# CIawevy/FreeFine

Hardware: NVIDIA B200
Metric: edits/s @512^2 50-step SD1.5 (FreeFine 2-D geometric edit) (higher is better)
Workload: dtype bf16

## Files before the change

freefine_b200/_lib.py:

```python
from __future__ import annotations

import ctypes as C
import os

_HERE = os.path.dirname(os.path.abspath(__file__))
LIB_PATH = os.environ.get("FREEFINE_B200_LIB", os.path.join(_HERE, "lib", "libfreefine_b200.so"))

FF_MAX_PASS = 4
FF_DT_F32, FF_DT_BF16, FF_DT_F16 = 0, 1, 2
FF_PASS_KEY_INVERT, FF_PASS_ROW_XOR, FF_PASS_ROW_WEIGHT, FF_PASS_KEY2_INVERT = 1, 2, 4, 8
FF_PASS_KEY_PREFIX, FF_PASS_KEY2_PREFIX = 16, 32


class FFAttnPass(C.Structure):
    _fields_ = [("kv_stream", C.c_int32), ("key_mask", C.c_int32), ("row_mask", C.c_int32), ("flags", C.c_uint32),
                ("weight", C.c_float), ("kv_stream2", C.c_int32), ("key_mask2", C.c_int32), ("reserved", C.c_int32)]


class FFAttnHeadPlan(C.Structure):
    _fields_ = [("n_pass", C.c_int32), ("reserved", C.c_int32 * 3), ("passes", FFAttnPass * FF_MAX_PASS)]


class FFAttnArgs(C.Structure):
    _fields_ = [("q", C.c_void_p), ("k", C.c_void_p), ("v", C.c_void_p), ("out", C.c_void_p), ("plan", C.c_void_p),
                ("bitmasks", C.c_void_p), ("mask_popcount", C.c_void_p),
                ("n_streams", C.c_int32), ("n_kv_streams", C.c_int32), ("heads", C.c_int32), ("head_dim", C.c_int32),
                ("s_q", C.c_int32), ("s_kv", C.c_int32), ("n_masks", C.c_int32), ("mask_words", C.c_int32),
                ("out_dtype", C.c_int32), ("scale", C.c_float), ("v_dtype", C.c_int32), ("v_head_stride", C.c_int32)]


PLAN_BYTES = C.sizeof(FFAttnHeadPlan)
PASS_BYTES = C.sizeof(FFAttnPass)

SIGNATURES = {
    "ff_version": (C.c_int, []),
    "ff_last_error": (C.c_char_p, []),
    "ff_attn_masked_kv": (C.c_int, [C.POINTER(FFAttnArgs), C.c_void_p]),
    "ff_attn_v_head_stride": (C.c_int, [C.c_int32]),
    "ff_attn_plain_smallkv": (C.c_int, [C.c_void_p] * 4 + [C.c_int32] * 5 + [C.c_float, C.c_int32, C.c_void_p]),
    "ff_debug_set_timeline": (C.c_int, [C.c_void_p]),
    "ff_kv_gather_cast": (C.c_int, [C.c_void_p, C.c_void_p, C.c_void_p, C.c_void_p, C.c_void_p, C.c_int32, C.c_int64,
                                    C.c_int32, C.c_int32, C.c_void_p]),
    "ff_mask_downsample_pack": (C.c_int, [C.c_void_p, C.c_int32, C.c_int32, C.c_int32, C.c_int32, C.c_int32,
                                          C.c_void_p, C.c_int32, C.c_void_p, C.c_void_p]),
    "ff_upsample2x_nhwc": (C.c_int, [C.c_void_p, C.c_void_p, C.c_int32, C.c_int32, C.c_int32, C.c_int32, C.c_void_p]),
    "ff_concat_nhwc": (C.c_int, [C.c_void_p, C.c_void_p, C.c_void_p, C.c_int64, C.c_int32, C.c_int32, C.c_void_p]),
    "ff_linear_bias_residual": (C.c_int, [C.c_void_p] * 5 + [C.c_int64, C.c_int32, C.c_int32, C.c_void_p, C.c_int64, C.c_void_p]),
    "ff_mask_prep": (C.c_int, [C.c_void_p] * 4 + [C.c_int32] * 7 + [C.c_void_p] * 6),
    "ff_dilate_mask": (C.c_int, [C.c_void_p, C.c_void_p, C.c_int32, C.c_int32, C.c_int32, C.c_int32, C.c_void_p]),
    "ff_warp_affine_blend": (C.c_int, [C.c_void_p, C.c_void_p, C.c_void_p, C.c_void_p, C.c_void_p, C.c_void_p,
                                       C.c_int32, C.c_int32, C.c_int32, C.c_int32, C.c_int32, C.c_int32, C.c_int32,
                                       C.c_int32, C.c_void_p]),
    "ff_ddim_cfg_step": (C.c_int, [C.c_void_p, C.c_void_p, C.c_void_p, C.c_void_p, C.c_void_p, C.c_float, C.c_float,
                                   C.c_float, C.c_float, C.c_float, C.c_float, C.c_float, C.c_void_p, C.c_void_p,
                                   C.c_int32, C.c_int32, C.c_int32, C.c_int32, C.c_void_p]),
    "ff_debug_set_trace": (C.c_int, [C.c_void_p]),
    "ff_ddim_step": (C.c_int, [C.c_void_p, C.c_void_p, C.c_void_p, C.c_void_p, C.c_float, C.c_float, C.c_float,
                               C.c_float, C.c_float, C.c_float, C.c_void_p, C.c_void_p, C.c_int32, C.c_int32,
                               C.c_int32, C.c_int32, C.c_void_p]),
    "ff_ddim_cfg_step_compose": (C.c_int, [C.c_void_p, C.c_int32, C.c_void_p, C.c_void_p, C.c_void_p, C.c_void_p,
                                           C.c_float, C.c_float, C.c_float, C.c_float, C.c_float, C.c_float, C.c_float,
                                           C.c_void_p, C.c_void_p, C.c_int32, C.c_int32, C.c_int32, C.c_int32, C.c_void_p]),
    "ff_ddim_inv_step": (C.c_int, [C.c_void_p, C.c_void_p, C.c_float, C.c_float, C.c_float, C.c_float, C.c_void_p,
                                   C.c_void_p, C.c_int64, C.c_void_p]),
    "ff_cross_region_blend": (C.c_int, [C.c_void_p, C.c_void_p, C.c_int32, C.c_void_p, C.c_int32, C.c_int32,
                                        C.c_int32, C.c_int32, C.c_void_p]),
    "ff_group_norm_ws_bytes": (C.c_int64, [C.c_int32, C.c_int32]),
    "ff_group_norm_nhwc": (C.c_int, [C.c_void_p, C.c_void_p, C.c_int64, C.c_void_p, C.c_void_p, C.c_void_p, C.c_void_p,
                                     C.c_int32, C.c_int32, C.c_int32, C.c_int32, C.c_float, C.c_int32, C.c_void_p]),
    "ff_bias_residual_nhwc": (C.c_int, [C.c_void_p, C.c_void_p, C.c_void_p, C.c_void_p, C.c_int64, C.c_int32,
                                        C.c_void_p]),
    "ff_geglu": (C.c_int, [C.c_void_p, C.c_void_p, C.c_int64, C.c_int32, C.c_void_p]),
    "ff_layer_norm": (C.c_int, [C.c_void_p, C.c_void_p, C.c_void_p, C.c_void_p, C.c_int64, C.c_int32, C.c_float,
                                C.c_void_p]),
}

_lib = None


def load() -> C.CDLL:
    global _lib
    if _lib is None:
        if not os.path.exists(LIB_PATH):
            raise RuntimeError(f"{LIB_PATH} is missing: build it with `python -m freefine_b200.csrc.build` "
                               "(freefine_b200 has no fallback path)")
        lib = C.CDLL(LIB_PATH)
        for name, (res, args) in SIGNATURES.items():
            fn = getattr(lib, name)
            fn.restype, fn.argtypes = res, args
        _lib = lib
    return _lib


def check(rc: int, what: str) -> None:
    if rc != 0:
        msg = load().ff_last_error()
        raise RuntimeError(f"{what} failed (code {rc}): {msg.decode() if msg else ''}")
```

freefine_b200/attention.py:

```python
from __future__ import annotations

import abc
import math

import os

import torch

from . import ops, plans


class AttentionControl(abc.ABC):
    def step_callback(self, x_t):
        return x_t

    def between_steps(self):
        return

    @property
    def num_uncond_att_layers(self):
        return self.num_att_layers if self.LOW_RESOURCE else 0

    @abc.abstractmethod
    def forward(self, attn, is_cross: bool, place_in_unet: str):
        raise NotImplementedError

    def _advance(self):
        self.cur_att_layer += 1
        if self.cur_att_layer == self.num_att_layers + self.num_uncond_att_layers:
            self.cur_att_layer = 0
            self.cur_step += 1
            self.between_steps()

    def __call__(self, attn, is_cross: bool, place_in_unet: str):
        self._advance()
        return attn

    def reset(self):
        self.cur_step = 0
        self.cur_att_layer = 0

    def __init__(self):
        self.cur_step = 0
        self.num_att_layers = -1
        self.cur_att_layer = 0
        self.LOW_RESOURCE = False


def _as_u8_stack(mask: torch.Tensor) -> torch.Tensor:
    m = mask if mask.dim() == 3 else mask[None]
    if m.dtype != torch.uint8:
        m = m.clamp(0, 255).to(torch.uint8)
    return m.contiguous()


class Attention_Modulator(AttentionControl):

    def __init__(self, start_layer=None):
        super().__init__()
        self.step_num = 0
        self.model_type = 'Inverse'
        self.use_cfg = False
        self.use_style_align = False
        self.use_tca = False
        self.local_edit = False
        self.fg_retain_mask = None
        self.fg_retain_mask_st2 = None
        self.fg_ref_mask = None
        self.obj_mask = None
        self.local_edit_region = None
        self.layer_idx = list(range(start_layer, 16)) if start_layer is not None else list(range(16))
        self.down_sampling_shape = dict()
        self.method = None
        self.context_guidance = None
        self.tca_scope = ['up']
        self.style_align_scope = ['down', 'mid', 'up']
        self.src_masks = None
        self.tgt_masks = None
        self.prompt_length = 1
        self.heads = None
        self.scale = None
        self.upcast_attention = False
        self.upcast_softmax = False
        self.log_mask = False
        self.sort_keys = True
        self.p_operand = "f16"
        self.small_kv_kernel = os.environ.get("FF_ATTN_SMALLKV", "1") != "0"
        self._tables = {}
        self._plans = {}

    def forward(self, attn, is_cross: bool, place_in_unet: str):
        return attn

    def reset(self):
        super().reset()
        self.step_num = 0
        self.model_type = 'Inverse'
        self.use_cfg = False
        self.use_tca = False
        self.use_style_align = False
        self.local_edit = False
        self.down_sampling_shape = dict()
        self.style_align = False
        self.method = None
        self.context_guidance = None
        self.tca_scope = ['up']
        self.style_align_scope = ['down', 'mid', 'up']
        self._tables.clear()
        self._plans.clear()

    def get_down_h_w(self, d_ratio, h, w, seq):
        if d_ratio in self.down_sampling_shape:
            nh, nw = self.down_sampling_shape[d_ratio]
            assert nh * nw == seq, f'{nh} * {nw} != {seq}'
            return nh, nw
        r = d_ratio // 8
        nh, nw = h // 8, w // 8
        while r != 1:
            r //= 2
            nh, nw = (nh + 1) // 2, (nw + 1) // 2
        assert nw * nh == seq
        self.down_sampling_shape[d_ratio] = [nh, nw]
        return nh, nw

    def _grid(self, H, W, seq):
        d_ratio = 2 ** int(math.log2((H * W // seq) ** 0.5) + 0.5)
        return self.get_down_h_w(d_ratio, H, W, seq)

    def _table(self, kind: str, seq: int, masks, min_tokens: int = 0):
        sig = tuple((m.data_ptr(), m._version, tuple(m.shape)) for m in masks)
        hit = self._tables.get((kind, seq))
        if hit is not None and hit[0] == sig:
            return hit[1], hit[2]
        stacks = [_as_u8_stack(m) for m in masks]
        E, H, W = stacks[0].shape
        for s in stacks:
            if s.shape != (E, H, W):
                raise ValueError(f"mask shapes differ: {[tuple(x.shape) for x in stacks]}")
            if not s.is_cuda:
                raise RuntimeError("controller masks must live on the CUDA device (no CPU path)")
        h, w = self._grid(H, W, seq)
        stacked = torch.stack(stacks, dim=1).reshape(E * len(stacks), H, W)
        words = ops.mask_words(max(seq, min_tokens))
        bits = torch.zeros((stacked.shape[0], words), dtype=torch.int32, device=stacked.device)
        bits, pop = ops.mask_downsample_pack(stacked, h, w, bits=bits)
        self._tables[(kind, seq)] = (sig, bits, pop, tuple(masks))
        return bits, pop

    def _plan(self, key, builder):
        p = self._plans.get(key)
        if p is None:
            if len(self._plans) > 256:
                self._plans.clear()
            host = builder()
            p = ops.to_device_bytes(host, self._device)
            self._plans[key] = p
            ops.PLAN_REGISTRY[p.data_ptr()] = host
        return p

    def _kv_index(self, kind: str, seq: int, bits, stream_masks):
        ck = (kind, "kvidx", seq)
        hit = self._tables.get(ck)
        if hit is not None and hit[0] is bits:
            return hit[1]
        shifts = torch.arange(32, device=bits.device, dtype=torch.int32)
        key_bits = ((bits[:, :, None] >> shifts) & 1).reshape(bits.shape[0], -1)[:, :seq]
        idx = plans.kv_sort_index(key_bits, stream_masks)
        self._tables[ck] = (bits, idx)
        return idx

    def _attend(self, query, key, value, plan, bits=None, pop=None, kv_index=None):
        self._device = query.device
        dt = query.dtype
        if dt not in (torch.float32, torch.bfloat16):
            query, key, value, dt = query.float(), key.float(), value.float(), torch.float32
        q = query.to(torch.bfloat16).contiguous()
        k = key.to(torch.bfloat16).contiguous()
        v = value.to(torch.bfloat16).contiguous()
        k, v = ops.kv_gather_cast(k, v, self.heads, kv_index, p_operand=self.p_operand)
        return ops.attn_masked_kv(q, k, v, plan, self.heads, self.scale, bits, pop, out_dtype=dt)

    def plain_attention(self, query, key, value):
        self._device = query.device
        B = query.shape[0]
        if key.shape[0] != B:
            raise ValueError("plain attention needs one K/V stream per query stream")
        d = query.shape[-1] // self.heads
        if (key.shape[1] <= (128 if d == 8 else ops.SMALLKV_MAX_KEYS) and d in ops.SMALLKV_HEAD_DIMS and self.p_operand == "f16"
                and self.small_kv_kernel):
            dt = query.dtype
            if dt not in (torch.float32, torch.bfloat16):
                query, key, value, dt = query.float(), key.float(), value.float(), torch.float32
            return ops.attn_plain_smallkv(query.to(torch.bfloat16).contiguous(), key.to(torch.bfloat16).contiguous(),
                                          value.to(torch.bfloat16).contiguous(), self.heads, self.scale, out_dtype=dt)
        plan = self._plan(("plain", B, self.heads), lambda: plans.plain_plan(B, self.heads))
        return self._attend(query, key, value, plan)

    def _tca_common(self, query, key, value, kind):
        B, S, _ = query.shape
        if self.cur_att_layer // 2 not in self.layer_idx:
            out = self.plain_attention(query, key, value)
            self._advance()
            return out
        if B % 4:
            raise ValueError(f"TCA expects 4 streams [u_e,u_r,c_e,c_r] per edit, got batch {B}")
        if self.method not in ('tca', 'mmsa'):
            raise ValueError(f"controller.method must be 'tca' or 'mmsa' here, got {self.method!r}")
        E = B // 4
        self._device = query.device
        if kind == "edit":
            bits, pop = self._table("edit", S, [self.fg_ref_mask, self.fg_retain_mask])
            src_id, tgt_id = (lambda e: 2 * e), (lambda e: 2 * e + 1)
        else:
            bits, pop = self._table("bg", S, [self.fg_retain_mask])
            src_id, tgt_id = (lambda e: e), (lambda e: e)
        if bits.shape[0] not in (2 * E if kind == "edit" else E,):
            raise ValueError(f"{E} edits in the stream batch but masks for {bits.shape[0]} rows")
        cg = None if self.method == 'mmsa' else float(self.context_guidance)
        pf = self.sort_keys
        plan = self._plan((kind, E, self.heads, self.method, cg, pf),
                          lambda: plans.tca_plan(E, self.heads, self.method, cg, src_id, tgt_id, kind=kind, prefix=pf))
        kv_index = None
        if pf:
            kv_index = self._kv_index(kind, S, bits, [src_id(s // 4) if s % 2 else -1 for s in range(B)])
        out = self._attend(query, key, value, plan, bits, pop, kv_index)
        self._advance()
        return out

    def Temporal_contextal_attention(self, query, key, value, is_cross, place_in_unet):
        return self._tca_common(query, key, value, "edit")

    def Temporal_contextal_attention_bg(self, query, key, value, is_cross, place_in_unet):
        return self._tca_common(query, key, value, "bg")

    def Temporal_contextal_attention_compose(self, query, key, value, is_cross, place_in_unet):
        B, S, _ = query.shape
        if self.cur_att_layer // 2 not in self.layer_idx:
            out = self.plain_attention(query, key, value)
            self._advance()
            return out
        N = B - 2
        self._device = query.device
        src = self.src_masks[:N] if torch.is_tensor(self.src_masks) else torch.stack(list(self.src_masks)[:N])
        tgt = self.tgt_masks[:N] if torch.is_tensor(self.tgt_masks) else torch.stack(list(self.tgt_masks)[:N])
        bits, pop = self._table("compose", S, [m for m in src] + [m for m in tgt])
        cg = None if self.method == 'mmsa' else float(self.context_guidance)
        pf = self.sort_keys
        plan = self._plan(("compose", N, self.heads, self.method, cg, pf),
                          lambda: plans.compose_plan(N, self.heads, self.method, cg, list(range(N)),
                                                     list(range(N, 2 * N)), prefix=pf))
        kv_index = self._kv_index("compose", S, bits, [-1] + list(range(N)) + [-1]) if pf else None
        out = self._attend(query, key, value, plan, bits, pop, kv_index)
        self._advance()
        return out

    def _style_align(self, query, key, value, mask, bg=False):
        B, S, _ = query.shape
        if B % 4:
            raise ValueError("style-align expects 4 streams per edit")
        E = B // 4
        self._device = query.device
        bits = pop = None
        src_id = None
        if self.method == 'sdsa':
            bits, pop = self._table("sdsa", S, [mask])
            src_id = lambda e: e
        pf = self.sort_keys and src_id is not None
        plan = self._plan(("style", E, self.heads, self.method, pf, bg),
                          lambda: plans.style_align_plan(E, self.heads, src_id, prefix=pf, bg=bg))
        kv_index = self._kv_index("sdsa", S, bits, [s // 4 if s % 2 else -1 for s in range(B)]) if pf else None
        out = self._attend(query, key, value, plan, bits, pop, kv_index)
        self._advance()
        return out

    def style_align_share_attention(self, query, key, value, is_cross, place_in_unet):
        return self._style_align(query, key, value, self.fg_ref_mask)

    def style_align_share_attention_bg(self, query, key, value, is_cross, place_in_unet):
        return self._style_align(query, key, value, self.fg_retain_mask, bg=True)

    def modulate_local_cross_attn(self, query, key, value, is_cross, place_in_unet):
        B, S, _ = query.shape
        if B % 4:
            raise ValueError("local cross-attention modulation expects 4 streams per edit")
        hs = self.plain_attention(query, key, value)
        bits, _ = self._table("region", S, [self.local_edit_region])
        ids = self._plans.get(("region_ids", B // 4))
        if ids is None:
            ids = torch.arange(B // 4, dtype=torch.int32, device=query.device)
            self._plans[("region_ids", B // 4)] = ids
        ops.cross_region_blend(hs, bits, ids)
        self._advance()
        return hs

    modulate_local_cross_attn_bg = modulate_local_cross_attn

    def modulate_local_cross_attn_compose(self, query, key, value, is_cross, place_in_unet):
        Bq, S, _ = query.shape
        self._device = query.device
        L = len(self.tgt_masks)
        nu = Bq - 1
        if key.shape[0] != nu + L:
            raise ValueError(f"expected {nu + L} prompt streams, got {key.shape[0]}")
        tg = self.tgt_masks if torch.is_tensor(self.tgt_masks) else torch.stack(list(self.tgt_masks))
        bits, pop = self._table("cross_compose", S, [m for m in tg], min_tokens=key.shape[1])

        def build():
            p = plans._empty(Bq, self.heads)
            for s in range(nu):
                for h in range(self.heads):
                    plans._add(p, s, h, s, 1.0)
            for h in range(self.heads):
                for i in range(L):
                    plans._add(p, nu, h, nu + i, 1.0, row_mask=i, flags=plans.FF_PASS_ROW_WEIGHT)
            return p

        plan = self._plan(("cross_compose", Bq, L, self.heads), build)
        out = self._attend(query, key, value, plan, bits, pop)
        self._advance()
        return out


def override_forward(unet):
    inner = unet.forward

    def forward(sample, timestep, encoder_hidden_states, *args, **kwargs):
        out = inner(sample, timestep, encoder_hidden_states, *args, **kwargs)
        if torch.is_tensor(out):
            return out
        return out.sample if hasattr(out, "sample") else out[0]

    return forward


class _DummyController:
    num_att_layers = 0
    use_tca = use_style_align = local_edit = False

    def __call__(self, *args):
        return args[0]


def _register(model, controller, flavour: str):
    if controller is None:
        controller = _DummyController()
    plain = Attention_Modulator()

    def ca_forward(self, place_in_unet):
        to_out = self.to_out[0] if isinstance(self.to_out, torch.nn.ModuleList) else self.to_out

        def forward(hidden_states, encoder_hidden_states=None, attention_mask=None, temb=None):
            is_cross = encoder_hidden_states is not None
            residual = hidden_states
            if self.spatial_norm is not None:
                hidden_states = self.spatial_norm(hidden_states, temb)
            input_ndim = hidden_states.ndim
            if input_ndim == 4:
                batch_size, channel, height, width = hidden_states.shape
                hidden_states = hidden_states.view(batch_size, channel, height * width).transpose(1, 2)
            if attention_mask is not None:
                raise NotImplementedError("explicit attention_mask is not part of the FreeFine hot path")
            if self.group_norm is not None:
                hidden_states = self.group_norm(hidden_states.transpose(1, 2)).transpose(1, 2)
            query = self.to_q(hidden_states)
            if encoder_hidden_states is None:
                encoder_hidden_states = hidden_states
            elif self.norm_cross:
                encoder_hidden_states = self.norm_encoder_hidden_states(encoder_hidden_states)
            key = self.to_k(encoder_hidden_states)
            value = self.to_v(encoder_hidden_states)

            c = controller if isinstance(controller, Attention_Modulator) else plain
            c.heads, c.scale = self.heads, self.scale
            c.upcast_attention, c.upcast_softmax = self.upcast_attention, self.upcast_softmax
            if flavour == "edit":
                if not is_cross and controller.use_style_align and place_in_unet in controller.style_align_scope:
                    hidden_states = controller.style_align_share_attention(query, key, value, is_cross, place_in_unet)
                elif not is_cross and controller.use_tca and place_in_unet in controller.tca_scope:
                    hidden_states = controller.Temporal_contextal_attention(query, key, value, is_cross, place_in_unet)
                elif controller.local_edit and is_cross:
                    hidden_states = controller.modulate_local_cross_attn(query, key, value, is_cross, place_in_unet)
                else:
                    hidden_states = c.plain_attention(query, key, value)
                    controller(None, is_cross, place_in_unet)
            elif flavour == "bggen":
                if place_in_unet in ['up'] and not is_cross and controller.use_tca:
                    hidden_states = controller.Temporal_contextal_attention_bg(query, key, value, is_cross, place_in_unet)
                elif controller.local_edit and is_cross:
                    hidden_states = controller.modulate_local_cross_attn_bg(query, key, value, is_cross, place_in_unet)
                else:
                    hidden_states = c.plain_attention(query, key, value)
                    controller(None, is_cross, place_in_unet)
            else:
                if not is_cross and controller.use_tca and place_in_unet in controller.tca_scope:
                    hidden_states = controller.Temporal_contextal_attention_compose(query, key, value, is_cross, place_in_unet)
                elif controller.local_edit and is_cross:
                    hidden_states = controller.modulate_local_cross_attn_compose(query, key, value, is_cross, place_in_unet)
                else:
                    hidden_states = c.plain_attention(query, key, value)
                    controller(None, is_cross, place_in_unet)

            block_res = getattr(self, "ff_block_residual", None)
            if (block_res is not None and input_ndim == 3 and hidden_states.is_cuda and hidden_states.dtype == torch.bfloat16
                    and isinstance(to_out, torch.nn.Linear) and not self.residual_connection
                    and self.rescale_output_factor == 1.0):
                self.ff_residual_fused = True
                return ops.linear_bias_residual(hidden_states.contiguous(), to_out.weight, to_out.bias, block_res)
            hidden_states = to_out(hidden_states)
            if input_ndim == 4:
                hidden_states = hidden_states.transpose(-1, -2).reshape(batch_size, channel, height, width)
            if self.residual_connection:
                hidden_states = hidden_states + residual
            if self.rescale_output_factor != 1.0:
                hidden_states = hidden_states / self.rescale_output_factor
            return hidden_states

        return forward

    def register_recr(net_, count, place_in_unet):
        if net_.__class__.__name__ == 'Attention':
            net_.forward = ca_forward(net_, place_in_unet)
            return count + 1
        if hasattr(net_, 'children'):
            for child in net_.children():
                count = register_recr(child, count, place_in_unet)
        return count

    n = 0
    for name, net in model.unet.named_children():
        if "down" in name:
            n += register_recr(net, 0, "down")
        elif "up" in name:
            n += register_recr(net, 0, "up")
        elif "mid" in name:
            n += register_recr(net, 0, "mid")
    controller.num_att_layers = n


def register_attention_control(model, controller):
    _register(model, controller, "edit")


def register_attention_control_4bggen(model, controller):
    _register(model, controller, "bggen")


def register_attention_control_compose(model, controller):
    _register(model, controller, "compose")
```

freefine_b200/csrc/cross_blend.cu:

```cuda
#include "ff_common.cuh"

namespace {

__global__ void __launch_bounds__(256)
cross_region_blend_kernel(uint4* __restrict__ hs, const uint32_t* __restrict__ bitmasks, int mask_words,
                          const int* __restrict__ region_mask, int n_edits, int S, int row_vec) {
  const long long per_stream = (long long)S * row_vec;
  const long long total = (long long)n_edits * per_stream;
  for (long long i = (long long)blockIdx.x * blockDim.x + threadIdx.x; i < total;
       i += (long long)gridDim.x * blockDim.x) {
    const int e = (int)(i / per_stream);
    const long long r = i - (long long)e * per_stream;
    const int tok = (int)(r / row_vec);
    const uint32_t word = __ldg(bitmasks + (size_t)__ldg(region_mask + e) * mask_words + (tok >> 5));
    const bool in_region = (word >> (tok & 31)) & 1u;
    uint4* base = hs + (long long)e * 4 * per_stream + r;
    const uint4 ur = base[per_stream];
    if (!in_region) base[2 * per_stream] = base[0];
    base[3 * per_stream] = ur;
  }
}

}

extern "C" int ff_cross_region_blend(void* hs, const uint32_t* bitmasks, int32_t mask_words,
                                     const int32_t* region_mask, int32_t n_edits, int32_t S, int32_t C, int32_t dtype,
                                     void* stream) {
  FF_REQUIRE(hs && bitmasks && region_mask, "ff_cross_region_blend: null pointer");
  FF_REQUIRE(n_edits > 0 && S > 0 && C > 0, "ff_cross_region_blend: bad shape");
  FF_REQUIRE(dtype == FF_DT_F32 || dtype == FF_DT_BF16, "ff_cross_region_blend: dtype must be f32 or bf16");
  const int es = dtype == FF_DT_F32 ? 4 : 2;
  FF_REQUIRE((C * es) % 16 == 0 && ff::aligned16(hs), "ff_cross_region_blend: rows must be 16-byte multiples");
  FF_REQUIRE(mask_words >= (S + 31) / 32, "ff_cross_region_blend: mask_words too small");
  const int row_vec = C * es / 16;
  const long long total = (long long)n_edits * S * row_vec;
  long long grid = (total + 255) / 256;
  if (grid > 148 * 8) grid = 148 * 8;
  cross_region_blend_kernel<<<(int)grid, 256, 0, static_cast<cudaStream_t>(stream)>>>(
      static_cast<uint4*>(hs), bitmasks, mask_words, region_mask, n_edits, S, row_vec);
  return ff::check_launch("ff_cross_region_blend");
}
```

freefine_b200/csrc/ddim_step.cu:

```cuda
#include "ff_common.cuh"

namespace {

struct StepCoef {
  float gs, sqrt_1m_at, sqrt_at, sqrt_ap, c_ddim, c_ddpm, sigma;
};

__device__ __forceinline__ void step_elem(float eu, float ec, float x, float nz, bool do_cfg, bool has_cfg_mask,
                                          uint8_t cfgm,
                                          uint8_t m, float sd, float cd, bool has_noise, const StepCoef& k,
                                          float& x_prev, float& x0) {
  float eps = eu;
  if (do_cfg) {
    float g = __fmul_rn(k.gs, __fsub_rn(ec, eu));
    if (has_cfg_mask) g = __fmul_rn(g, (float)cfgm);
    eps = __fadd_rn(eu, g);
  }
  x0 = __fdiv_rn(__fsub_rn(x, __fmul_rn(k.sqrt_1m_at, eps)), k.sqrt_at);
  const uint8_t om = (uint8_t)(1 - m);
  const float pdm = __fmul_rn(__fmul_rn(cd, eps), (float)m);
  const float dir = __fadd_rn(__fmul_rn(__fmul_rn(k.c_ddim, eps), (float)om), pdm);
  float xp = __fadd_rn(__fmul_rn(k.sqrt_ap, x0), dir);
  if (has_noise) xp = __fadd_rn(xp, __fmul_rn(__fmul_rn(sd, nz), (float)m));
  x_prev = xp;
}

template <int V>
__global__ void __launch_bounds__(256)
ddim_cfg_step_kernel(const float* __restrict__ eps4, const float* __restrict__ x, const float* __restrict__ noise,
                     const uint8_t* __restrict__ cfg_mask, const uint8_t* __restrict__ var_mask, StepCoef k,
                     float* __restrict__ x_prev, float* __restrict__ pred_x0, int n_edits, int C, int hw, int spe,
                     int so, int cs) {
  const int hwv = hw / V;
  const long long total = (long long)n_edits * so * C * hwv;
  for (long long i = (long long)blockIdx.x * blockDim.x + threadIdx.x; i < total;
       i += (long long)gridDim.x * blockDim.x) {
    const int p = (int)(i % hwv);
    long long r = i / hwv;
    const int c = (int)(r % C);
    r /= C;
    const int s = so == 2 ? (int)(r & 1) : 0;
    const int e = so == 2 ? (int)(r >> 1) : (int)r;
    const long long off_u = (((long long)(e * spe + s) * C + c) * hw) + (long long)p * V;
    const long long off_c = (((long long)(e * spe + s + cs) * C + c) * hw) + (long long)p * V;
    const long long off_x = (((long long)(e * so + s) * C + c) * hw) + (long long)p * V;
    const long long off_m = (long long)e * hw + (long long)p * V;
    float eu[V], ec[V], xv[V], nz[V], xp[V], x0[V];
    uint8_t cm[V], vm[V];
    if (V == 4) {
      *reinterpret_cast<float4*>(eu) = __ldg(reinterpret_cast<const float4*>(eps4 + off_u));
      *reinterpret_cast<float4*>(ec) = __ldg(reinterpret_cast<const float4*>(eps4 + off_c));
      *reinterpret_cast<float4*>(xv) = __ldg(reinterpret_cast<const float4*>(x + off_x));
      if (noise) *reinterpret_cast<float4*>(nz) = __ldg(reinterpret_cast<const float4*>(noise + off_x));
      if (cfg_mask) *reinterpret_cast<uint32_t*>(cm) = __ldg(reinterpret_cast<const uint32_t*>(cfg_mask + off_m));
      if (s == 0) *reinterpret_cast<uint32_t*>(vm) = __ldg(reinterpret_cast<const uint32_t*>(var_mask + off_m));
    } else {
      eu[0] = __ldg(eps4 + off_u);
      ec[0] = __ldg(eps4 + off_c);
      xv[0] = __ldg(x + off_x);
      if (noise) nz[0] = __ldg(noise + off_x);
      if (cfg_mask) cm[0] = __ldg(cfg_mask + off_m);
      if (s == 0) vm[0] = __ldg(var_mask + off_m);
    }
    const float sd = s == 0 ? k.sigma : 0.f;
    const float cd = s == 0 ? k.c_ddpm : k.c_ddim;
#pragma unroll
    for (int j = 0; j < V; ++j) {
      const uint8_t m = s == 0 ? vm[j] : (uint8_t)1;
      step_elem(eu[j], ec[j], xv[j], noise ? nz[j] : 0.f, cs != 0, cfg_mask != nullptr, cfg_mask ? cm[j] : (uint8_t)1,
                m, sd, cd, noise != nullptr, k, xp[j], x0[j]);
    }
    if (V == 4) {
      *reinterpret_cast<float4*>(x_prev + off_x) = *reinterpret_cast<float4*>(xp);
      if (pred_x0) *reinterpret_cast<float4*>(pred_x0 + off_x) = *reinterpret_cast<float4*>(x0);
    } else {
      x_prev[off_x] = xp[0];
      if (pred_x0) pred_x0[off_x] = x0[0];
    }
  }
}

template <int V>
__global__ void __launch_bounds__(256)
ddim_inv_step_kernel(const float* __restrict__ eps, const float* __restrict__ x, float sqrt_1m_at, float sqrt_at,
                     float sqrt_an, float c_next, float* __restrict__ x_next, float* __restrict__ pred_x0,
                     long long nv) {
  for (long long i = (long long)blockIdx.x * blockDim.x + threadIdx.x; i < nv;
       i += (long long)gridDim.x * blockDim.x) {
    float e[V], xv[V], xn[V], x0[V];
    if (V == 4) {
      *reinterpret_cast<float4*>(e) = __ldg(reinterpret_cast<const float4*>(eps) + i);
      *reinterpret_cast<float4*>(xv) = __ldg(reinterpret_cast<const float4*>(x) + i);
    } else {
      e[0] = __ldg(eps + i);
      xv[0] = __ldg(x + i);
    }
#pragma unroll
    for (int j = 0; j < V; ++j) {
      x0[j] = __fdiv_rn(__fsub_rn(xv[j], __fmul_rn(sqrt_1m_at, e[j])), sqrt_at);
      xn[j] = __fadd_rn(__fmul_rn(sqrt_an, x0[j]), __fmul_rn(c_next, e[j]));
    }
    if (V == 4) {
      reinterpret_cast<float4*>(x_next)[i] = *reinterpret_cast<float4*>(xn);
      if (pred_x0) reinterpret_cast<float4*>(pred_x0)[i] = *reinterpret_cast<float4*>(x0);
    } else {
      x_next[i] = xn[0];
      if (pred_x0) pred_x0[i] = x0[0];
    }
  }
}

inline int grid_for(long long work_items, int block) {
  long long need = (work_items + block - 1) / block;
  const long long cap = 148LL * 8;
  if (need > cap) need = cap;
  if (need < 1) need = 1;
  return (int)need;
}

}

static int launch_step(const char* what, const float* eps, int spe, int so, int cs, const float* x, const float* noise,
                       const uint8_t* cfg_mask, const uint8_t* var_mask, const StepCoef& k, float* x_prev,
                       float* pred_x0, int32_t n_edits, int32_t C, int32_t h, int32_t w, void* stream) {
  if (!(eps && x && var_mask && x_prev)) return ff::fail(FF_E_INVALID, "%s: null pointer", what);
  if (!(n_edits > 0 && C > 0 && h > 0 && w > 0))
    return ff::fail(FF_E_INVALID, "%s: bad shape %d,%d,%d,%d", what, n_edits, C, h, w);
  const int hw = h * w;
  cudaStream_t st = static_cast<cudaStream_t>(stream);
  const bool vec = (hw % 4 == 0) && ff::aligned16(eps) && ff::aligned16(x) && ff::aligned16(x_prev) &&
                   (!noise || ff::aligned16(noise)) && (!pred_x0 || ff::aligned16(pred_x0)) &&
                   (reinterpret_cast<uintptr_t>(var_mask) % 4 == 0) &&
                   (!cfg_mask || reinterpret_cast<uintptr_t>(cfg_mask) % 4 == 0);
  if (vec) {
    const long long items = (long long)n_edits * so * C * (hw / 4);
    ddim_cfg_step_kernel<4><<<grid_for(items, 256), 256, 0, st>>>(eps, x, noise, cfg_mask, var_mask, k, x_prev,
                                                                   pred_x0, n_edits, C, hw, spe, so, cs);
  } else {
    const long long items = (long long)n_edits * so * C * hw;
    ddim_cfg_step_kernel<1><<<grid_for(items, 256), 256, 0, st>>>(eps, x, noise, cfg_mask, var_mask, k, x_prev,
                                                                   pred_x0, n_edits, C, hw, spe, so, cs);
  }
  return ff::check_launch(what);
}

extern "C" int ff_ddim_cfg_step(const float* eps4, const float* x, const float* noise, const uint8_t* cfg_mask,
                                const uint8_t* var_mask, float guidance_scale, float sqrt_1m_at, float sqrt_at,
                                float sqrt_ap, float c_ddim, float c_ddpm, float sigma, float* x_prev,
                                float* pred_x0, int32_t n_edits, int32_t C, int32_t h, int32_t w, void* stream) {
  StepCoef k{guidance_scale, sqrt_1m_at, sqrt_at, sqrt_ap, c_ddim, c_ddpm, sigma};
  return launch_step("ff_ddim_cfg_step", eps4, 4, 2, 2, x, noise, cfg_mask, var_mask, k, x_prev, pred_x0, n_edits, C, h,
                     w, stream);
}

extern "C" int ff_ddim_step(const float* eps2, const float* x, const float* noise, const uint8_t* var_mask,
                            float sqrt_1m_at, float sqrt_at, float sqrt_ap, float c_ddim, float c_ddpm, float sigma,
                            float* x_prev, float* pred_x0, int32_t n_edits, int32_t C, int32_t h, int32_t w,
                            void* stream) {
  StepCoef k{0.f, sqrt_1m_at, sqrt_at, sqrt_ap, c_ddim, c_ddpm, sigma};
  return launch_step("ff_ddim_step", eps2, 2, 2, 0, x, noise, nullptr, var_mask, k, x_prev, pred_x0, n_edits, C, h, w,
                     stream);
}

extern "C" int ff_ddim_cfg_step_compose(const float* eps, int32_t streams_per_edit, const float* x, const float* noise,
                                        const uint8_t* cfg_mask, const uint8_t* var_mask, float guidance_scale,
                                        float sqrt_1m_at, float sqrt_at, float sqrt_ap, float c_ddim, float c_ddpm,
                                        float sigma, float* x_prev, float* pred_x0, int32_t n_edits, int32_t C, int32_t h,
                                        int32_t w, void* stream) {
  FF_REQUIRE(streams_per_edit >= 2, "ff_ddim_cfg_step_compose: streams_per_edit=%d < 2", streams_per_edit);
  StepCoef k{guidance_scale, sqrt_1m_at, sqrt_at, sqrt_ap, c_ddim, c_ddpm, sigma};
  return launch_step("ff_ddim_cfg_step_compose", eps, streams_per_edit, 1, streams_per_edit - 1, x, noise, cfg_mask,
                     var_mask, k, x_prev, pred_x0, n_edits, C, h, w, stream);
}

extern "C" int ff_ddim_inv_step(const float* eps, const float* x, float sqrt_1m_at, float sqrt_at, float sqrt_an,
                                float c_next, float* x_next, float* pred_x0, int64_t n, void* stream) {
  FF_REQUIRE(eps && x && x_next, "ff_ddim_inv_step: null pointer");
  FF_REQUIRE(n > 0, "ff_ddim_inv_step: n must be positive");
  cudaStream_t st = static_cast<cudaStream_t>(stream);
  const bool vec = (n % 4 == 0) && ff::aligned16(eps) && ff::aligned16(x) && ff::aligned16(x_next) &&
                   (!pred_x0 || ff::aligned16(pred_x0));
  if (vec) {
    ddim_inv_step_kernel<4><<<grid_for(n / 4, 256), 256, 0, st>>>(eps, x, sqrt_1m_at, sqrt_at, sqrt_an, c_next,
                                                                   x_next, pred_x0, n / 4);
  } else {
    ddim_inv_step_kernel<1><<<grid_for(n, 256), 256, 0, st>>>(eps, x, sqrt_1m_at, sqrt_at, sqrt_an, c_next, x_next,
                                                               pred_x0, n);
  }
  return ff::check_launch("ff_ddim_inv_step");
}
```

freefine_b200/ops.py:

```python
from __future__ import annotations

import contextlib
import ctypes as C
import os

import numpy as np
import torch

from . import _lib
from ._lib import FF_DT_BF16, FF_DT_F32

_DT = {torch.float32: FF_DT_F32, torch.bfloat16: FF_DT_BF16}

COUNTS: dict = {}
PROFILE = None
PLAN_REGISTRY: dict = {}


NVTX = os.environ.get("FREEFINE_NVTX", "0") == "1"


@contextlib.contextmanager
def nvtx_range(name: str):
    if NVTX and torch.cuda.is_available():
        torch.cuda.nvtx.range_push(name)
        try:
            yield
        finally:
            torch.cuda.nvtx.range_pop()
    else:
        yield


LIBRARY_ENTRIES = frozenset({"ff_linear_bias_residual"})


def _count(name: str):
    COUNTS[name] = COUNTS.get(name, 0) + 1


_RAW_STREAM = getattr(torch._C, "_cuda_getCurrentRawStream", None)


def _stream() -> C.c_void_p:
    if _RAW_STREAM is not None:
        return C.c_void_p(_RAW_STREAM(torch.cuda.current_device()))
    return C.c_void_p(torch.cuda.current_stream().cuda_stream)


def _ptr(t):
    return None if t is None else C.c_void_p(t.data_ptr())


def _chk(t: torch.Tensor, dtype, name: str, dims=None):
    if not t.is_cuda:
        raise RuntimeError(f"{name} must be a CUDA tensor (freefine_b200 has no CPU path)")
    if t.dtype != dtype:
        raise TypeError(f"{name} must be {dtype}, got {t.dtype}")
    if not t.is_contiguous():
        raise ValueError(f"{name} must be contiguous")
    if dims is not None and t.dim() != dims:
        raise ValueError(f"{name} must have {dims} dims, got {tuple(t.shape)}")
    return t


def ddim_cfg_step(eps4, x, noise, cfg_mask, var_mask, guidance_scale, sqrt_1m_at, sqrt_at, sqrt_ap, c_ddim, c_ddpm,
                  sigma, want_pred_x0=False, out=None):
    _chk(eps4, torch.float32, "eps4")
    _chk(x, torch.float32, "x")
    Cc, h, w = x.shape[-3:]
    n_edits = x.numel() // (2 * Cc * h * w)
    if eps4.numel() != 2 * x.numel():
        raise ValueError(f"eps4 {tuple(eps4.shape)} must hold 4 streams per edit for x {tuple(x.shape)}")
    _chk(var_mask, torch.uint8, "var_mask")
    if var_mask.numel() != n_edits * h * w:
        raise ValueError("var_mask must be [n_edits,h,w]")
    if cfg_mask is not None:
        _chk(cfg_mask, torch.uint8, "cfg_mask")
        if cfg_mask.numel() != n_edits * h * w:
            raise ValueError("cfg_mask must be [n_edits,h,w]")
    if noise is not None:
        _chk(noise, torch.float32, "noise")
        if noise.numel() != x.numel():
            raise ValueError("noise must have the shape of x")
    x_prev = torch.empty_like(x) if out is None else _chk(out, torch.float32, "out")
    x0 = torch.empty_like(x) if want_pred_x0 else None
    lib = _lib.load()
    rc = lib.ff_ddim_cfg_step(_ptr(eps4), _ptr(x), _ptr(noise), _ptr(cfg_mask), _ptr(var_mask), guidance_scale,
                              sqrt_1m_at, sqrt_at, sqrt_ap, c_ddim, c_ddpm, sigma, _ptr(x_prev), _ptr(x0), n_edits,
                              Cc, h, w, _stream())
    _lib.check(rc, "ff_ddim_cfg_step")
    _count("ff_ddim_cfg_step")
    return (x_prev, x0) if want_pred_x0 else x_prev


def ddim_step(eps2, x, noise, var_mask, sqrt_1m_at, sqrt_at, sqrt_ap, c_ddim, c_ddpm, sigma, want_pred_x0=False):
    _chk(eps2, torch.float32, "eps2")
    _chk(x, torch.float32, "x")
    if eps2.shape != x.shape:
        raise ValueError("eps2 and x must have the same shape")
    Cc, h, w = x.shape[-3:]
    n_edits = x.numel() // (2 * Cc * h * w)
    _chk(var_mask, torch.uint8, "var_mask")
    if var_mask.numel() != n_edits * h * w:
        raise ValueError("var_mask must be [n_edits,h,w]")
    if noise is not None:
        _chk(noise, torch.float32, "noise")
    x_prev = torch.empty_like(x)
    x0 = torch.empty_like(x) if want_pred_x0 else None
    rc = _lib.load().ff_ddim_step(_ptr(eps2), _ptr(x), _ptr(noise), _ptr(var_mask), sqrt_1m_at, sqrt_at, sqrt_ap,
                                  c_ddim, c_ddpm, sigma, _ptr(x_prev), _ptr(x0), n_edits, Cc, h, w, _stream())
    _lib.check(rc, "ff_ddim_step")
    _count("ff_ddim_step")
    return (x_prev, x0) if want_pred_x0 else x_prev


def ddim_cfg_step_compose(eps, streams_per_edit, x, noise, cfg_mask, var_mask, guidance_scale, sqrt_1m_at, sqrt_at,
                          sqrt_ap, c_ddim, c_ddpm, sigma):
    _chk(eps, torch.float32, "eps")
    _chk(x, torch.float32, "x")
    Cc, h, w = x.shape[-3:]
    E = x.numel() // (Cc * h * w)
    if eps.numel() != E * streams_per_edit * Cc * h * w:
        raise ValueError("eps must hold streams_per_edit streams per edit")
    _chk(var_mask, torch.uint8, "var_mask")
    if cfg_mask is not None:
        _chk(cfg_mask, torch.uint8, "cfg_mask")
    if noise is not None:
        _chk(noise, torch.float32, "noise")
    x_prev = torch.empty_like(x)
    rc = _lib.load().ff_ddim_cfg_step_compose(_ptr(eps), streams_per_edit, _ptr(x), _ptr(noise), _ptr(cfg_mask), _ptr(var_mask),
                                              guidance_scale, sqrt_1m_at, sqrt_at, sqrt_ap, c_ddim, c_ddpm, sigma,
                                              _ptr(x_prev), None, E, Cc, h, w, _stream())
    _lib.check(rc, "ff_ddim_cfg_step_compose")
    _count("ff_ddim_cfg_step_compose")
    return x_prev


def ddim_inv_step(eps, x, sqrt_1m_at, sqrt_at, sqrt_an, c_next, want_pred_x0=False):
    _chk(eps, torch.float32, "eps")
    _chk(x, torch.float32, "x")
    if eps.shape != x.shape:
        raise ValueError("eps and x must have the same shape")
    x_next = torch.empty_like(x)
    x0 = torch.empty_like(x) if want_pred_x0 else None
    rc = _lib.load().ff_ddim_inv_step(_ptr(eps), _ptr(x), sqrt_1m_at, sqrt_at, sqrt_an, c_next, _ptr(x_next), _ptr(x0),
                                      x.numel(), _stream())
    _lib.check(rc, "ff_ddim_inv_step")
    _count("ff_ddim_inv_step")
    return (x_next, x0) if want_pred_x0 else x_next


def warp_affine_blend(src, theta, dsize=None, mask_src=None, bg=None, mode="bilinear", want_mask=False, out=None):
    if src.dtype not in _DT:
        raise TypeError(f"src must be float32 or bfloat16, got {src.dtype}")
    _chk(src, src.dtype, "src", 4)
    N, Cc, H, W = src.shape
    dW, dH = (W, H) if dsize is None else dsize
    theta = theta.to(device=src.device, dtype=torch.float32)
    if theta.dim() == 2:
        theta = theta[None].expand(N, 2, 3)
    theta = theta.contiguous()
    if theta.shape != (N, 2, 3):
        raise ValueError(f"theta must be [N,2,3], got {tuple(theta.shape)}")
    if mask_src is not None:
        _chk(mask_src, torch.uint8, "mask_src")
        if mask_src.numel() != N * H * W:
            raise ValueError("mask_src must be [N,H,W]")
        if bg is None:
            raise ValueError("mask_src needs a background")
        _chk(bg, src.dtype, "bg", 4)
        if bg.shape != (N, Cc, dH, dW):
            raise ValueError("bg must be [N,C,dH,dW]")
    if out is None:
        out = torch.empty((N, Cc, dH, dW), dtype=src.dtype, device=src.device)
    else:
        _chk(out, src.dtype, "out", 4)
        if out.shape != (N, Cc, dH, dW):
            raise ValueError("out must be [N,C,dH,dW]")
    mask_out = torch.empty((N, dH, dW), dtype=torch.uint8, device=src.device) if (want_mask and mask_src is not None) else None
    rc = _lib.load().ff_warp_affine_blend(_ptr(src), _ptr(theta), _ptr(mask_src), _ptr(bg), _ptr(out), _ptr(mask_out),
                                          N, Cc, H, W, dH, dW, 0 if mode == "bilinear" else 1, _DT[src.dtype],
                                          _stream())
    _lib.check(rc, "ff_warp_affine_blend")
    _count("ff_warp_affine_blend")
    return (out, mask_out) if want_mask else out


def mask_words(S: int) -> int:
    return (S + 31) // 32


def mask_downsample_pack(masks, h, w, bits=None, popcount=None):
    _chk(masks, torch.uint8, "masks", 3)
    n, H, W = masks.shape
    words = mask_words(h * w)
    if bits is None:
        bits = torch.empty((n, words), dtype=torch.int32, device=masks.device)
    if popcount is None:
        popcount = torch.empty((n,), dtype=torch.int32, device=masks.device)
    rc = _lib.load().ff_mask_downsample_pack(_ptr(masks), n, H, W, h, w, _ptr(bits), bits.shape[1], _ptr(popcount),
                                             _stream())
    _lib.check(rc, "ff_mask_downsample_pack")
    _count("ff_mask_downsample_pack")
    return bits, popcount


def mask_prep(shifted, ori, draw, cons, lat_hw, use_auto_draw, reduce_inp_artifacts):
    _chk(shifted, torch.uint8, "shifted", 3)
    _chk(ori, torch.uint8, "ori", 3)
    E, H, W = shifted.shape
    for name, t in (("ori", ori), ("draw", draw), ("cons", cons)):
        if t is not None:
            _chk(t, torch.uint8, name, 3)
            if tuple(t.shape) != (E, H, W):
                raise ValueError(f"{name} must be [{E},{H},{W}], got {tuple(t.shape)}")
    h, w = lat_hw
    dev = shifted.device
    fg, sh, orib = (torch.empty((E, H, W), dtype=torch.uint8, device=dev) for _ in range(3))
    comp, lvar = (torch.empty((E, h, w), dtype=torch.uint8, device=dev) for _ in range(2))
    rc = _lib.load().ff_mask_prep(_ptr(shifted), _ptr(ori), _ptr(draw), _ptr(cons), E, H, W, h, w, int(bool(use_auto_draw)),
                                  int(bool(reduce_inp_artifacts)), _ptr(fg), _ptr(sh), _ptr(orib), _ptr(comp), _ptr(lvar), _stream())
    _lib.check(rc, "ff_mask_prep")
    _count("ff_mask_prep")
    return fg, sh, orib, comp, lvar


def dilate_mask(mask, k):
    m = mask if mask.dim() == 3 else mask[None]
    _chk(m, torch.uint8, "mask", 3)
    out = torch.empty_like(m)
    rc = _lib.load().ff_dilate_mask(_ptr(m), _ptr(out), m.shape[0], m.shape[1], m.shape[2], int(k), _stream())
    _lib.check(rc, "ff_dilate_mask")
    _count("ff_dilate_mask")
    return out if mask.dim() == 3 else out[0]


class StagedV:
    __slots__ = ("data", "heads", "head_dim")

    def __init__(self, data, heads, head_dim):
        self.data, self.heads, self.head_dim = data, heads, head_dim

    def values(self):
        return self.data[..., : self.head_dim].reshape(self.data.shape[0], self.data.shape[1], -1)


P_OPERAND_DTYPE = {"f16": torch.float16, "bf16x2": torch.bfloat16}


def kv_gather_cast(k, v, heads, row_index=None, gather_k=True, p_operand="f16"):
    _chk(k, torch.bfloat16, "k", 3)
    _chk(v, torch.bfloat16, "v", 3)
    if v.shape != k.shape or k.shape[2] % heads:
        raise ValueError("k and v must have the same shape [Bk,Skv,heads*d]")
    Bk, Sk, Ck = k.shape
    d = Ck // heads
    if row_index is not None:
        _chk(row_index, torch.int64, "row_index", 1)
        if row_index.numel() != Bk * Sk:
            raise ValueError("row_index must hold one source row per K/V row")
    lib = _lib.load()
    vhs = lib.ff_attn_v_head_stride(d)
    do_k = gather_k and row_index is not None
    k_out = torch.empty_like(k) if do_k else None
    vdt = P_OPERAND_DTYPE[p_operand]
    v_out = torch.empty((Bk, Sk, heads, vhs), dtype=vdt, device=v.device)
    rc = lib.ff_kv_gather_cast(_ptr(k) if do_k else None, _ptr(v), _ptr(row_index), _ptr(k_out), _ptr(v_out),
                               _lib.FF_DT_F16 if vdt == torch.float16 else FF_DT_BF16, Bk * Sk, heads, d, _stream())
    _lib.check(rc, "ff_kv_gather_cast")
    _count("ff_kv_gather_cast")
    return (k_out if do_k else k), StagedV(v_out, heads, d)


def attn_masked_kv(q, k, v, plan, heads, scale, bitmasks=None, popcount=None, out_dtype=None, out=None,
                   p_operand="f16"):
    _chk(q, torch.bfloat16, "q", 3)
    _chk(k, torch.bfloat16, "k", 3)
    B, Sq, Cc = q.shape
    Bk, Skv, Ck = k.shape
    if Ck != Cc or Cc % heads:
        raise ValueError(f"bad shapes q{tuple(q.shape)} k{tuple(k.shape)} heads={heads}")
    if not isinstance(v, StagedV):
        _chk(v, torch.bfloat16, "v", 3)
        if v.shape != k.shape:
            raise ValueError(f"bad shapes k{tuple(k.shape)} v{tuple(v.shape)}")
        v = kv_gather_cast(k, v, heads, None, p_operand=p_operand)[1]
    vt = v.data
    _chk(vt, vt.dtype if vt.dtype in (torch.float16, torch.bfloat16) else torch.float16, "v", 4)
    if tuple(vt.shape[:3]) != (Bk, Skv, heads) or v.head_dim * heads != Ck:
        raise ValueError(f"staged V {tuple(vt.shape)} does not match k{tuple(k.shape)} heads={heads}")
    _chk(plan, torch.uint8, "plan")
    if plan.numel() != B * heads * _lib.PLAN_BYTES:
        raise ValueError(f"plan holds {plan.numel()} bytes, expected {B * heads * _lib.PLAN_BYTES}")
    out_dtype = torch.bfloat16 if out_dtype is None else out_dtype
    if out is None:
        out = torch.empty((B, Sq, Cc), dtype=out_dtype, device=q.device)
    else:
        _chk(out, out_dtype, "out", 3)
    a = _lib.FFAttnArgs()
    a.q, a.k, a.v, a.out, a.plan = q.data_ptr(), k.data_ptr(), vt.data_ptr(), out.data_ptr(), plan.data_ptr()
    if bitmasks is not None:
        _chk(bitmasks, torch.int32, "bitmasks", 2)
        _chk(popcount, torch.int32, "popcount", 1)
        a.bitmasks, a.mask_popcount = bitmasks.data_ptr(), popcount.data_ptr()
        a.n_masks, a.mask_words = bitmasks.shape[0], bitmasks.shape[1]
    else:
        a.bitmasks, a.mask_popcount, a.n_masks, a.mask_words = None, None, 0, 0
    a.n_streams, a.n_kv_streams, a.heads, a.head_dim = B, Bk, heads, Cc // heads
    a.s_q, a.s_kv = Sq, Skv
    a.out_dtype = _DT[out_dtype]
    a.scale = float(scale)
    a.v_dtype = _lib.FF_DT_F16 if vt.dtype == torch.float16 else FF_DT_BF16
    a.v_head_stride = vt.shape[3]
    prof = PROFILE
    if prof is not None:
        ev0, ev1 = torch.cuda.Event(enable_timing=True), torch.cuda.Event(enable_timing=True)
        ev0.record()
    with nvtx_range(f"ff_attn_masked_kv S_q={Sq} S_kv={Skv} d={Cc // heads} streams={B}"):
        rc = _lib.load().ff_attn_masked_kv(C.byref(a), _stream())
    _lib.check(rc, "ff_attn_masked_kv")
    COUNTS["ff_attn_masked_kv"] = COUNTS.get("ff_attn_masked_kv", 0) + 1
    if prof is not None:
        ev1.record()
        prof.append(dict(ev0=ev0, ev1=ev1, B=B, Bk=Bk, s_q=Sq, s_kv=Skv, d=Cc // heads, heads=heads, plan=PLAN_REGISTRY.get(plan.data_ptr()),
                         popcount=popcount))
    return out


SMALLKV_MAX_KEYS = 256
SMALLKV_HEAD_DIMS = (8, 40, 80, 160)


def attn_plain_smallkv(q, k, v, heads, scale, out_dtype=None):
    _chk(q, torch.bfloat16, "q", 3)
    _chk(k, torch.bfloat16, "k", 3)
    _chk(v, torch.bfloat16, "v", 3)
    B, Sq, Cc = q.shape
    if k.shape[0] != B or k.shape[2] != Cc or v.shape != k.shape or Cc % heads:
        raise ValueError(f"bad shapes q{tuple(q.shape)} k{tuple(k.shape)} v{tuple(v.shape)} heads={heads}")
    out_dtype = torch.bfloat16 if out_dtype is None else out_dtype
    out = torch.empty((B, Sq, Cc), dtype=out_dtype, device=q.device)
    with nvtx_range(f"ff_attn_plain_smallkv S_q={Sq} S_kv={k.shape[1]} d={Cc // heads} streams={B}"):
        rc = _lib.load().ff_attn_plain_smallkv(_ptr(q), _ptr(k), _ptr(v), _ptr(out), B, heads, Cc // heads, Sq, k.shape[1],
                                               float(scale), _DT[out_dtype], _stream())
    _lib.check(rc, "ff_attn_plain_smallkv")
    _count("ff_attn_plain_smallkv")
    return out


def cross_region_blend(hs, bitmasks, region_ids):
    if hs.dtype not in _DT:
        raise TypeError("hs must be float32 or bfloat16")
    _chk(hs, hs.dtype, "hs", 3)
    B, S, Cc = hs.shape
    if B % 4:
        raise ValueError("hs must hold 4 streams per edit")
    _chk(bitmasks, torch.int32, "bitmasks", 2)
    _chk(region_ids, torch.int32, "region_ids", 1)
    rc = _lib.load().ff_cross_region_blend(_ptr(hs), _ptr(bitmasks), bitmasks.shape[1], _ptr(region_ids), B // 4, S, Cc,
                                           _DT[hs.dtype], _stream())
    _lib.check(rc, "ff_cross_region_blend")
    _count("ff_cross_region_blend")
    return hs


def _nhwc_view(x: torch.Tensor, name: str):
    if not x.is_cuda:
        raise RuntimeError(f"{name} must be a CUDA tensor (freefine_b200 has no CPU path)")
    if x.dtype != torch.bfloat16:
        raise TypeError(f"{name} must be bfloat16, got {x.dtype}")
    if x.dim() != 4:
        raise ValueError(f"{name} must be [N,C,H,W], got {tuple(x.shape)}")
    if not x.permute(0, 2, 3, 1).is_contiguous():
        raise ValueError(f"{name} must be dense channels_last (NHWC) memory")
    N, Cc, H, W = x.shape
    return N, H * W, Cc


_GN_WS: dict = {}


def _gn_workspace(N: int, G: int, device) -> torch.Tensor:
    key = (device, _stream().value)
    need = int(_lib.load().ff_group_norm_ws_bytes(N, G))
    ws = _GN_WS.get(key)
    if ws is None or ws.numel() < need:
        ws = torch.zeros(max(need, 1 << 20), dtype=torch.uint8, device=device)
        _GN_WS[key] = ws
    return ws


def group_norm_nhwc(x, gamma, beta, groups, eps, add_nc=None, silu=False):
    N, HW, Cc = _nhwc_view(x, "x")
    _chk(gamma, torch.bfloat16, "gamma", 1)
    _chk(beta, torch.bfloat16, "beta", 1)
    if gamma.numel() != Cc or beta.numel() != Cc:
        raise ValueError("gamma / beta must have C elements")
    add_ld = Cc
    if add_nc is not None:
        if not add_nc.is_cuda or add_nc.dtype != torch.float32 or add_nc.dim() != 2:
            raise TypeError("add_nc must be a 2-D float32 CUDA tensor")
        if tuple(add_nc.shape) != (N, Cc) or add_nc.stride(1) != 1 or (N > 1 and add_nc.stride(0) < Cc):
            raise ValueError(f"add_nc must be [{N},{Cc}] with unit column stride, got {tuple(add_nc.shape)} {add_nc.stride()}")
        add_ld = add_nc.stride(0) if N > 1 else Cc
    y = torch.empty_like(x)
    ws = _gn_workspace(N, groups, x.device)
    rc = _lib.load().ff_group_norm_nhwc(_ptr(x), _ptr(add_nc), add_ld, _ptr(gamma), _ptr(beta), _ptr(y), _ptr(ws), N, HW, Cc,
                                        groups, float(eps), int(bool(silu)), _stream())
    _lib.check(rc, "ff_group_norm_nhwc")
    _count("ff_group_norm_nhwc")
    return y


def bias_residual_nhwc(h, bias=None, res=None):
    N, HW, Cc = _nhwc_view(h, "h")
    if bias is not None:
        _chk(bias, torch.bfloat16, "bias", 1)
        if bias.numel() != Cc:
            raise ValueError("bias must have C elements")
    if res is not None:
        if _nhwc_view(res, "res") != (N, HW, Cc):
            raise ValueError("res must have the shape of h")
    rc = _lib.load().ff_bias_residual_nhwc(_ptr(h), _ptr(bias), _ptr(res), _ptr(h), N * HW, Cc, _stream())
    _lib.check(rc, "ff_bias_residual_nhwc")
    _count("ff_bias_residual_nhwc")
    return h


def upsample2x_nhwc(x):
    N, HW, Cc = _nhwc_view(x, "x")
    H, W = x.shape[2], x.shape[3]
    y = torch.empty((N, Cc, 2 * H, 2 * W), dtype=x.dtype, device=x.device, memory_format=torch.channels_last)
    rc = _lib.load().ff_upsample2x_nhwc(_ptr(x), _ptr(y), N, H, W, Cc, _stream())
    _lib.check(rc, "ff_upsample2x_nhwc")
    _count("ff_upsample2x_nhwc")
    return y


def concat_nhwc(a, b):
    N, HW, Ca = _nhwc_view(a, "a")
    Nb, HWb, Cb = _nhwc_view(b, "b")
    if (N, HW) != (Nb, HWb) or a.shape[2:] != b.shape[2:]:
        raise ValueError(f"concat_nhwc: shapes {tuple(a.shape)} and {tuple(b.shape)} differ outside the channel dimension")
    out = torch.empty((N, Ca + Cb, a.shape[2], a.shape[3]), dtype=a.dtype, device=a.device, memory_format=torch.channels_last)
    rc = _lib.load().ff_concat_nhwc(_ptr(a), _ptr(b), _ptr(out), N * HW, Ca, Cb, _stream())
    _lib.check(rc, "ff_concat_nhwc")
    _count("ff_concat_nhwc")
    return out


_LT_WS: dict = {}


def linear_bias_residual(x, weight, bias=None, res=None, out=None):
    _chk(x, torch.bfloat16, "x")
    _chk(weight, torch.bfloat16, "weight", 2)
    N, K = weight.shape
    if x.shape[-1] != K:
        raise ValueError(f"x has {x.shape[-1]} features, weight expects {K}")
    M = x.numel() // K
    if bias is not None:
        _chk(bias, torch.bfloat16, "bias", 1)
        if bias.numel() != N:
            raise ValueError("bias must have N elements")
    oshape = tuple(x.shape[:-1]) + (N,)
    if res is not None:
        _chk(res, torch.bfloat16, "res")
        if tuple(res.shape) != oshape:
            raise ValueError(f"res must be {oshape}, got {tuple(res.shape)}")
    if out is None:
        out = torch.empty(oshape, dtype=torch.bfloat16, device=x.device)
    else:
        _chk(out, torch.bfloat16, "out")
        if tuple(out.shape) != oshape:
            raise ValueError(f"out must be {oshape}, got {tuple(out.shape)}")
    key = (x.device, _stream().value)
    ws = _LT_WS.get(key)
    if ws is None:
        ws = _LT_WS[key] = torch.empty(32 << 20, dtype=torch.uint8, device=x.device)
    rc = _lib.load().ff_linear_bias_residual(_ptr(x), _ptr(weight), _ptr(bias), _ptr(res), _ptr(out), M, N, K, _ptr(ws),
                                             ws.numel(), _stream())
    _lib.check(rc, "ff_linear_bias_residual")
    _count("ff_linear_bias_residual")
    return out


def geglu(h):
    _chk(h, torch.bfloat16, "h")
    F2 = h.shape[-1]
    if F2 % 2:
        raise ValueError("last dim must be even")
    M = h.numel() // F2
    out = torch.empty(*h.shape[:-1], F2 // 2, dtype=h.dtype, device=h.device)
    rc = _lib.load().ff_geglu(_ptr(h), _ptr(out), M, F2 // 2, _stream())
    _lib.check(rc, "ff_geglu")
    _count("ff_geglu")
    return out


def layer_norm(x, gamma, beta, eps):
    _chk(x, torch.bfloat16, "x")
    Cc = x.shape[-1]
    _chk(gamma, torch.bfloat16, "gamma", 1)
    _chk(beta, torch.bfloat16, "beta", 1)
    if gamma.numel() != Cc or beta.numel() != Cc:
        raise ValueError("gamma / beta must have C elements")
    y = torch.empty_like(x)
    rc = _lib.load().ff_layer_norm(_ptr(x), _ptr(gamma), _ptr(beta), _ptr(y), x.numel() // Cc, Cc, float(eps), _stream())
    _lib.check(rc, "ff_layer_norm")
    _count("ff_layer_norm")
    return y


def to_device_bytes(arr: np.ndarray, device) -> torch.Tensor:
    t = torch.from_numpy(np.ascontiguousarray(arr).view(np.uint8).reshape(-1))
    if torch.cuda.is_available():
        t = t.pin_memory()
    return t.to(device, non_blocking=True)
```

freefine_b200/pipeline.py:

```python
from __future__ import annotations

from copy import deepcopy

import numpy as np
import torch
import torch.nn.functional as F

from . import ops
from .attention import (Attention_Modulator, override_forward, register_attention_control,
                        register_attention_control_4bggen, register_attention_control_compose)


def randn_tensor(shape, generator=None, device=None, dtype=None):
    return torch.randn(tuple(shape), generator=generator, device=device, dtype=dtype)


def seed_everything(seed):
    torch.manual_seed(seed)
    np.random.seed(seed % (2 ** 32))
    return seed


class FreeFinePipeline:

    def __init__(self, unet, vae, tokenizer, text_encoder, scheduler, controller=None, device=None):
        self.unet, self.vae, self.tokenizer = unet, vae, tokenizer
        self.text_encoder, self.scheduler = text_encoder, scheduler
        self.controller = controller
        self._device = torch.device(device) if device is not None else next(unet.parameters()).device
        self.method_type = None

    @classmethod
    def from_parts(cls, parts, controller=None, device=None):
        return cls(parts.unet, parts.vae, parts.tokenizer, parts.text_encoder, parts.scheduler, controller, device)

    @property
    def device(self):
        return self._device

    def modify_unet_forward(self):
        self.unet.forward = override_forward(self.unet)

    def _ratio(self):
        return self.scheduler.config.num_train_timesteps // self.scheduler.num_inference_steps

    def _get_variance(self, timestep, prev_timestep):
        a_t = self.scheduler.alphas_cumprod[timestep]
        a_prev = self.scheduler.alphas_cumprod[prev_timestep] if prev_timestep >= 0 else self.scheduler.final_alpha_cumprod
        return ((1 - a_prev) / (1 - a_t)) * (1 - a_t / a_prev)

    def _ctrl_coefs(self, timestep, eta):
        t = int(timestep)
        prev_t = t - self._ratio()
        a_t = self.scheduler.alphas_cumprod[t]
        a_prev = self.scheduler.alphas_cumprod[prev_t] if prev_t > 0 else self.scheduler.final_alpha_cumprod
        std = eta * self._get_variance(t, prev_t).to(torch.float32) ** 0.5
        stdt = torch.cat((std[None,], torch.zeros_like(std)[None,]))
        c_ddpm = ((1 - a_prev - stdt ** 2) ** 0.5)[0]
        return dict(sqrt_1m_at=float((1 - a_t) ** 0.5), sqrt_at=float(a_t ** 0.5), sqrt_ap=float(a_prev ** 0.5),
                    c_ddim=float((1 - a_prev) ** 0.5), c_ddpm=float(c_ddpm), sigma=float(std))

    def _inv_coefs(self, timestep):
        nxt = int(timestep)
        t = min(nxt - self._ratio(), 999)
        a_t = self.scheduler.alphas_cumprod[t] if t >= 0 else self.scheduler.final_alpha_cumprod
        a_next = self.scheduler.alphas_cumprod[nxt]
        return dict(sqrt_1m_at=float((1 - a_t) ** 0.5), sqrt_at=float(a_t ** 0.5), sqrt_an=float(a_next ** 0.5),
                    c_next=float((1 - a_next) ** 0.5))

    def inv_step(self, model_output, timestep, x, eta=0., verbose=False):
        return ops.ddim_inv_step(model_output.float().contiguous(), x.float().contiguous(), want_pred_x0=True,
                                 **self._inv_coefs(timestep))

    def _var_mask(self, mask, n_edits, h, w):
        m = mask
        if m.dtype != torch.uint8:
            raise TypeError(f"ctrl_step mask must be uint8 (reference quirk Q2), got {m.dtype}")
        m = m.reshape(-1, h, w)
        if m.shape[0] == 1 and n_edits > 1:
            m = m.expand(n_edits, h, w)
        if m.shape[0] != n_edits:
            raise ValueError(f"mask for {m.shape[0]} edits, latents for {n_edits}")
        return m.contiguous().to(self.device)

    def ctrl_step(self, model_output, timestep, x, mask, eta: float = 0.0, generator=None):
        if model_output.shape[0] % 2 or mask is None:
            raise NotImplementedError("ctrl_step mirrors the 2-stream [edit, ref] local-DDPM form of the reference")
        E = model_output.shape[0] // 2
        h, w = x.shape[-2:]
        noise = None
        if eta > 0:
            noise = randn_tensor(model_output.shape, generator=generator, device=model_output.device,
                                 dtype=torch.float32).contiguous()
        return ops.ddim_step(model_output.float().contiguous(), x.float().contiguous(), noise,
                             self._var_mask(mask, E, h, w), want_pred_x0=True, **self._ctrl_coefs(timestep, eta))

    def cfg_ctrl_step(self, noise_pred4, timestep, x, cfg_mask, var_mask, guidance_scale, eta=0.0, generator=None):
        E = x.shape[0] // 2
        h, w = x.shape[-2:]
        noise = None
        if eta > 0:
            if isinstance(generator, (list, tuple)):
                if len(generator) != E:
                    raise ValueError(f"{len(generator)} generators for {E} edits")
                noise = torch.stack([randn_tensor((2,) + tuple(x.shape[1:]), generator=g, device=x.device, dtype=torch.float32)
                                     for g in generator]).reshape(x.shape).contiguous()
            else:
                noise = randn_tensor(x.shape, generator=generator, device=x.device, dtype=torch.float32).contiguous()
        cm = None if cfg_mask is None else self._var_mask(cfg_mask, E, h, w)
        return ops.ddim_cfg_step(noise_pred4.float().contiguous(), x.float().contiguous(), noise, cm,
                                 self._var_mask(var_mask, E, h, w), float(guidance_scale),
                                 **self._ctrl_coefs(timestep, eta))

    def linear_param(self, t, t1, t0, t2, end_scale=0.5):
        if t < t1 or t > t2:
            raise ValueError(f"t must be in [{t1}, {t2}]")
        if t <= t0:
            return 1 + (end_scale - 1) / (t0 - t1) * (t - t1)
        return end_scale + (-end_scale / (t2 - t0)) * (t - t0)

    def preprocess_image(self, image, device):
        image = torch.from_numpy(image).float() / 127.5 - 1
        return image.permute(2, 0, 1).unsqueeze(0).to(device)

    @torch.no_grad()
    def image2latent(self, image):
        if isinstance(image, np.ndarray):
            if image.dtype == np.uint8:
                image = image.astype(np.float32) / 255.0 * 2 - 1
            image = torch.from_numpy(image)
        tensor = image.clone().detach()
        if tensor.ndim == 3:
            tensor = tensor.permute(2, 0, 1).unsqueeze(0)
        elif tensor.ndim != 4:
            raise ValueError(f"Invalid tensor shape: {tensor.shape}")
        tensor = tensor.to(device=self.device, dtype=next(self.vae.parameters()).dtype)
        return self.vae.encode(tensor)['latent_dist'].mean * 0.18215

    @torch.no_grad()
    def latent2image(self, latents, return_type='np'):
        latents = 1 / 0.18215 * latents.detach()
        image = self.vae.decode(latents.to(next(self.vae.parameters()).dtype))['sample']
        image = (image.float() / 2 + 0.5).clamp(0, 1)
        if return_type == 'np':
            image = (image.cpu().permute(0, 2, 3, 1).numpy()[0] * 255).astype(np.uint8)
        return image

    @torch.no_grad()
    def get_text_embeddings(self, prompt):
        ids = self.tokenizer(prompt, padding="max_length", max_length=77, return_tensors="pt").input_ids
        return self.text_encoder(ids.to(self.device))[0]

    def _unet(self, latents, t, text_embeddings):
        dt = self.unet.dtype if hasattr(self.unet, "dtype") else next(self.unet.parameters()).dtype
        if latents.is_cuda and not (torch.is_tensor(t) and t.is_cuda):
            t = torch.full((), int(t), dtype=torch.int64, device=latents.device)
        with ops.nvtx_range(f"ff.unet streams={latents.shape[0]}"):
            out = self.unet(latents.to(dt), t, encoder_hidden_states=text_embeddings.to(dt))
        return out.float()

    @torch.no_grad()
    def invert(self, image, prompt, num_inference_steps=50, num_actual_inference_steps=None, guidance_scale=7.5,
               eta=0.0, return_intermediates=False, verbose=False, **kwds):
        batch_size = image.shape[0]
        if isinstance(prompt, list):
            if batch_size == 1:
                image = image.expand(len(prompt), -1, -1, -1)
        elif isinstance(prompt, str) and batch_size > 1:
            prompt = [prompt] * batch_size
        text_embeddings = self.get_text_embeddings(prompt)
        latents = self.image2latent(image).float()
        if guidance_scale > 1.:
            uncond = self.get_text_embeddings([""] * batch_size)
            text_embeddings = torch.cat([uncond, text_embeddings], dim=0)
            self.controller.use_cfg = True
        self.scheduler.set_timesteps(num_inference_steps)
        latents_list = [latents]
        for i, t in enumerate(reversed(self.scheduler.timesteps)):
            if num_actual_inference_steps is not None and i >= num_actual_inference_steps:
                continue
            with ops.nvtx_range(f"ff.invert step {i} t={int(t)}"):
                model_inputs = torch.cat([latents] * 2) if guidance_scale > 1. else latents
                noise_pred = self._unet(model_inputs, t, text_embeddings)
                if guidance_scale > 1.:
                    eu, ec = noise_pred.chunk(2, dim=0)
                    noise_pred = eu + guidance_scale * (ec - eu)
                latents, _ = self.inv_step(noise_pred, t, latents)
            latents_list.append(latents)
        if return_intermediates:
            return latents, latents_list
        return latents

    @torch.no_grad()
    def forward_sampling(self, prompt, prompt_embeds=None, refer_latents=None, batch_size=1, end_step=None,
                         height=512, width=512, num_inference_steps=50, num_actual_inference_steps=None,
                         guidance_scale=7.5, latents=None, unconditioning=None, neg_prompt=None,
                         return_intermediates=False, eta=0.0, end_scale=0.5, local_var_reg=None,
                         completion_mask_cfg=None, local_edit_text=True, share_attn=True, method_type=None,
                         verbose=False, local_perturbation=True, generator=None, **kwds):
        self.method_type = method_type
        assert guidance_scale > 1.0, 'USING THIS MODULE CFG Must > 1.0'
        c = self.controller
        if share_attn:
            if method_type == 'tca':
                c.use_tca, c.layer_idx, c.method = True, list(range(10, 16)), 'tca'
            elif method_type in ('mmsa', 'mmsa_es'):
                c.use_tca, c.layer_idx, c.method = True, list(range(10, 16)), 'mmsa'
            elif method_type == 'ssa':
                c.use_style_align, c.method = True, 'ssa'
            elif method_type == 'sdsa':
                c.use_style_align, c.method = True, 'sdsa'
        c.use_cfg = True
        c.local_edit = local_edit_text
        if prompt_embeds is None:
            if isinstance(prompt, str) and batch_size > 1:
                prompt = [prompt] * batch_size
            cond = self.get_text_embeddings(prompt)
        else:
            cond = prompt_embeds
        n2 = cond.shape[0]
        if n2 % 2:
            raise ValueError("forward_sampling expects [edit_prompt, \"\"] pairs")
        E = n2 // 2
        if latents is None:
            latents = torch.randn((n2, self.unet.in_channels, height // 8, width // 8), device=self.device)
        uncond = self.get_text_embeddings([neg_prompt if neg_prompt else ""] * n2)
        text_embeddings = torch.cat([uncond.reshape(E, 2, *uncond.shape[1:]), cond.reshape(E, 2, *cond.shape[1:])],
                                    dim=1).reshape(4 * E, *cond.shape[1:])
        self.scheduler.set_timesteps(num_inference_steps)
        latents = latents.float().clone()
        latents_list = [latents]
        if num_actual_inference_steps is None:
            num_actual_inference_steps = num_inference_steps
        start_step = num_inference_steps - num_actual_inference_steps
        C, h, w = latents.shape[1:]
        var_mask = local_var_reg if local_perturbation else torch.ones_like(local_var_reg)
        for i, t in enumerate(self.scheduler.timesteps):
            if i < start_step:
                continue
            ref_latent = refer_latents[i - start_step + 1].reshape(E, 2, C, h, w)[:, 1]
            if latents.shape[0] == 2 * E:
                latents = latents.clone()
                latents.view(E, 2, C, h, w)[:, 1] = ref_latent
            else:
                latents = torch.stack([latents.reshape(E, C, h, w), ref_latent], 1).reshape(2 * E, C, h, w)
            if method_type == 'tca':
                c.context_guidance = self.linear_param(i, start_step, end_step, num_inference_steps, end_scale=end_scale)
            elif method_type == 'mmsa_es' and i >= end_step:
                c.use_tca = False
            lat = latents.view(E, 2, C, h, w)
            model_inputs = torch.cat([lat, lat], dim=1).reshape(4 * E, C, h, w)
            te = text_embeddings
            if unconditioning is not None and isinstance(unconditioning, list):
                te = text_embeddings.clone().reshape(E, 4, *cond.shape[1:])
                te[:, :2] = unconditioning[i].to(te.dtype)
                te = te.reshape(4 * E, *cond.shape[1:])
            c.log_mask = False
            with ops.nvtx_range(f"ff.sample step {i} t={int(t)}"):
                noise_pred = self._unet(model_inputs, t, te)
                latents = self.cfg_ctrl_step(noise_pred, t, latents, completion_mask_cfg if local_edit_text else None,
                                             var_mask, guidance_scale, eta=eta, generator=generator)
            latents_list.append(latents)
        image = self.latent2image(latents, return_type="pt")
        if return_intermediates:
            return image, latents_list
        return image, None

    def mask_reduce_dim(self, mask):
        return mask[:, :, 0] if mask.ndim == 3 else mask

    def dilate_mask(self, mask, dilate_factor=15):
        k = int(dilate_factor)
        a = k // 2
        m = torch.from_numpy(np.ascontiguousarray(mask.astype(np.uint8))).to(self.device)
        squeeze = m.dim() == 2
        if m.is_cuda and m.shape[1] % 4 == 0 and int(m.max()) <= 1:
            y = ops.dilate_mask(m if squeeze else m.permute(2, 0, 1).contiguous(), k)
            return (y if squeeze else y.permute(1, 2, 0)).cpu().numpy()
        x = (m[None, None] if squeeze else m.permute(2, 0, 1)[None]).float()
        x = F.pad(x, (a, k - 1 - a, a, k - 1 - a), value=0.0)
        y = F.max_pool2d(x, kernel_size=k, stride=1)
        y = y[0, 0] if squeeze else y[0].permute(1, 2, 0)
        return y.to(torch.uint8).cpu().numpy()

    def prepare_tensor_mask(self, mask, sup_res_w, sup_res_h, binary=True):
        if mask.ndim == 3:
            mask = mask[:, :, 0]
        t = torch.tensor(mask, device=self.device)[None, None]
        t = F.interpolate(t, (sup_res_h, sup_res_w), mode="nearest").squeeze(0).squeeze(0)
        if binary:
            t[t > 0.0] = 1.0
        else:
            norm_ = t.max()
            t = t.float()
            t /= norm_
        return t

    def _masks_for_kernel(self, masks, sup_res_w, sup_res_h, init_code):
        if self.device.type != 'cuda':
            return None
        lh, lw = init_code.shape[2], init_code.shape[3]
        if sup_res_h % lh or sup_res_w % lw or sup_res_w % 4:
            return None
        out = []
        for m in masks:
            if m is None:
                out.append(None)
                continue
            m = np.asarray(m)
            m = m[:, :, 0] if m.ndim == 3 else m
            if m.shape != (sup_res_h, sup_res_w) or m.dtype.kind not in 'ub':
                return None
            out.append(torch.from_numpy(np.ascontiguousarray(m.astype(np.uint8)))[None].to(self.device))
        return out

    def prepare_various_mask(self, shifted_mask, ori_mask, draw_mask, sup_res_w, sup_res_h, init_code, verbose=False,
                             use_auto_draw=False, cons_area=None, reduce_inp_artifacts=False):
        if use_auto_draw or reduce_inp_artifacts:
            assert cons_area is not None, 'for auto draw / auto artifact expansion use cons area '
        dev_masks = self._masks_for_kernel((shifted_mask, ori_mask, None if use_auto_draw else draw_mask,
                                            cons_area if (use_auto_draw or reduce_inp_artifacts) else None),
                                           sup_res_w, sup_res_h, init_code)
        if dev_masks is not None:
            r = ops.mask_prep(*dev_masks, (init_code.shape[2], init_code.shape[3]), use_auto_draw, reduce_inp_artifacts)
            return tuple(t[0] for t in r)
        P = lambda m: self.prepare_tensor_mask(m, sup_res_w, sup_res_h)
        if not use_auto_draw:
            if not reduce_inp_artifacts:
                sh, ori = P(shifted_mask), P(ori_mask)
                flex = P(draw_mask) * (1 - sh)
                fg = flex + sh
                fg[fg > 0] = 1.0
                comp, lvar = flex, flex
            else:
                assert cons_area is not None, 'for auto artifact expansion use cons area '
                dil = P(self.dilate_mask(ori_mask, 30))
                cons, sh, ori = P(cons_area), P(shifted_mask), P(ori_mask)
                flex = P(draw_mask) * (1 - sh)
                fg = flex + sh
                fg[fg > 0] = 1.0
                comp = flex
                lvar = (1 - cons) * (1 - sh) * dil + flex
                lvar[lvar > 0] = 1
        else:
            assert cons_area is not None, 'for auto draw better use cons area '
            if not reduce_inp_artifacts:
                dil_t = P(self.dilate_mask(shifted_mask, 15))
                sh, ori, cons = P(shifted_mask), P(ori_mask), P(cons_area)
                fg = sh
                cons = cons - ori
                comp = (1 - cons) * (1 - sh) * dil_t
                lvar = comp
            else:
                dil_t = P(self.dilate_mask(shifted_mask, 15))
                dil = P(self.dilate_mask(ori_mask, 30))
                sh, ori, cons = P(shifted_mask), P(ori_mask), P(cons_area)
                fg = sh
                cons = cons - ori
                comp = dil + dil_t
                comp[comp > 0] = 1
                comp *= (1 - cons) * (1 - sh)
                lvar = comp
        size = (init_code.shape[2], init_code.shape[3])
        comp = F.interpolate(comp[None, None], size, mode='nearest').squeeze(0).squeeze(0)
        lvar = F.interpolate(lvar[None, None], size, mode='nearest').squeeze(0).squeeze(0)
        return fg, sh, ori, comp, lvar

    @torch.no_grad()
    def DDIM_inversion_func(self, img, mask, prompt, num_step, start_step=0, ref_img=None, verbose=False):
        source_image = self.preprocess_image(img, self.device)
        if ref_img is not None:
            source_image = torch.cat((source_image, self.preprocess_image(ref_img, self.device)))
        if mask.ndim == 3:
            mask = mask[:, :, 0]
        latents, latents_list = self.invert(source_image, prompt, guidance_scale=1.0, num_inference_steps=num_step,
                                            num_actual_inference_steps=num_step - start_step,
                                            return_intermediates=True, verbose=verbose)
        self.controller.reset()
        return np.asarray(mask, dtype=np.float32), latents_list

    def Details_Preserving_regeneration(self, source_image, inverted_latents, edit_prompt, shifted_mask, ori_mask,
                                        draw_mask, num_steps=100, start_step=30, end_step=10, eta=1,
                                        guidance_scale=7.5, share_attn=True, method_type='tca', verbose=False,
                                        local_text_edit=True, local_perturbation=True, return_intermediates=False,
                                        use_auto_draw=False, cons_area=None, use_share_attention=False,
                                        reduce_inp_artifacts=False, end_scale=0.5):
        start_latents = inverted_latents[-1]
        init_code_orig = deepcopy(start_latents)
        full_h, full_w = source_image.shape[:2]
        fg_retain, fg_retain_st2, fg_ref, comp_cfg, local_var = self.prepare_various_mask(
            shifted_mask, ori_mask, draw_mask, full_h, full_w, init_code_orig, verbose=verbose,
            use_auto_draw=use_auto_draw, cons_area=cons_area, reduce_inp_artifacts=reduce_inp_artifacts)
        c = self.controller
        c.fg_retain_mask = fg_retain.to(self.device)
        c.fg_retain_mask_st2 = fg_retain_st2.to(self.device)
        c.fg_ref_mask = fg_ref.to(self.device)
        c.local_edit_region = fg_retain.to(self.device)
        c.reset()
        c.log_mask = False
        gen_images, intermediates = self.forward_sampling(
            prompt=[edit_prompt, ""], refer_latents=inverted_latents[::-1], end_step=end_step, batch_size=2,
            latents=init_code_orig, guidance_scale=guidance_scale, num_inference_steps=num_steps,
            num_actual_inference_steps=num_steps - start_step, eta=eta, completion_mask_cfg=comp_cfg,
            local_var_reg=local_var, share_attn=share_attn, method_type=method_type, verbose=verbose,
            blending=local_text_edit, local_perturbation=local_perturbation, return_intermediates=return_intermediates,
            use_share_attention=use_share_attention, end_scale=end_scale)
        edit_gen_image, ref_gen_image = gen_images
        c.reset()
        to_u8 = lambda im: (im.permute(1, 2, 0).detach().cpu().numpy() * 255).astype(np.uint8)
        return to_u8(edit_gen_image), to_u8(ref_gen_image), intermediates

    def FreeFine_generation(self, ori_img, ori_mask, coarse_input, target_mask, guidance_text, guidance_scale, eta,
                            end_step=10, num_step=50, start_step=25, share_attn=True, method_type='tca',
                            local_text_edit=True, local_perturbation=True, verbose=True, return_ori=False, seed=42,
                            draw_mask=None, return_intermediates=False, use_auto_draw=False, cons_area=None,
                            reduce_inp_artifacts=False, end_scale=0.5):
        methods = ['tca', 'ssa', 'sdsa', 'mmsa', 'mmsa_es']
        assert method_type in methods, f"check method type f{method_type}, which is not in {methods}"
        seed_everything(seed)
        ori_mask = self.mask_reduce_dim(ori_mask)
        target_mask = self.mask_reduce_dim(target_mask)
        if draw_mask is not None:
            draw_mask = self.mask_reduce_dim(draw_mask)
        shifted_mask, inverted_latent = self.DDIM_inversion_func(img=coarse_input, mask=target_mask, prompt="",
                                                                 num_step=num_step, start_step=start_step,
                                                                 ref_img=ori_img, verbose=verbose)
        edit_img, ref_img, intermediates = self.Details_Preserving_regeneration(
            coarse_input, inverted_latent, guidance_text, target_mask, ori_mask, draw_mask, num_steps=num_step,
            start_step=start_step, end_step=end_step, guidance_scale=guidance_scale, eta=eta, share_attn=share_attn,
            method_type=method_type, verbose=verbose, local_text_edit=local_text_edit,
            local_perturbation=local_perturbation, return_intermediates=return_intermediates, cons_area=cons_area,
            use_auto_draw=use_auto_draw, end_scale=end_scale, reduce_inp_artifacts=reduce_inp_artifacts)
        self.last_intermediates = intermediates
        if not return_ori:
            return edit_img
        return edit_img, ref_img


    def prepare_mask_bggen(self, mask, sup_res_w, sup_res_h, init_code):
        mask_tensor = self.prepare_tensor_mask(mask, sup_res_w, sup_res_h)
        lvar = F.interpolate(mask_tensor[None, None], (init_code.shape[2], init_code.shape[3]), mode='nearest')
        return mask_tensor, lvar.squeeze(0).squeeze(0)

    @torch.no_grad()
    def forward_sampling_background_gen(self, prompt, batch_size=1, end_step=None, height=512, width=512,
                                        num_inference_steps=50, num_actual_inference_steps=None, guidance_scale=7.5,
                                        latents=None, refer_latents=None, unconditioning=None, neg_prompt=None,
                                        return_intermediates=False, eta=0.0, local_var_reg=None, local_cfg_reg=None,
                                        local_text_edit=True, share_attn=True, method_type='tca', verbose=False,
                                        local_perturbation=True, end_scale=0.5, latent_blended=True,
                                        blend_range=(0, 40), **kwds):
        assert guidance_scale > 1.0, 'USING THIS MODULE CFG Must > 1.0'
        self.method_type = method_type
        c = self.controller
        if share_attn:
            if method_type == 'tca':
                c.use_tca, c.layer_idx, c.method = True, list(range(10, 16)), 'tca'
            elif method_type in ('mmsa', 'mmsa_es'):
                c.use_tca, c.layer_idx, c.method = True, list(range(10, 16)), 'mmsa'
            elif method_type == 'ssa':
                c.use_style_align, c.method = True, 'ssa'
            elif method_type == 'sdsa':
                c.use_style_align, c.method = True, 'sdsa'
        c.use_cfg = True
        c.local_edit = local_text_edit
        if isinstance(prompt, str) and batch_size > 1:
            prompt = [prompt] * batch_size
        cond = self.get_text_embeddings(prompt)
        n2 = cond.shape[0]
        E = n2 // 2
        uncond = self.get_text_embeddings([neg_prompt if neg_prompt else ""] * n2)
        text_embeddings = torch.cat([uncond.reshape(E, 2, *uncond.shape[1:]), cond.reshape(E, 2, *cond.shape[1:])],
                                    dim=1).reshape(4 * E, *cond.shape[1:])
        self.scheduler.set_timesteps(num_inference_steps)
        if num_actual_inference_steps is None:
            num_actual_inference_steps = num_inference_steps
        start_step = num_inference_steps - num_actual_inference_steps
        C, h, w = latents.shape[1:]
        edit = latents.float().reshape(-1, C, h, w)[:E] if latents.shape[0] == E else latents.float().reshape(E, -1, C, h, w)[:, 0]
        latents_list = [latents]
        var_mask = local_var_reg if local_perturbation else torch.ones_like(local_var_reg)
        for i, t in enumerate(self.scheduler.timesteps):
            if i < start_step:
                continue
            ref = refer_latents[i - start_step].float().reshape(E, C, h, w)
            lat = torch.stack([edit, ref], dim=1)
            if method_type == 'tca':
                c.context_guidance = self.linear_param(i, start_step, end_step, num_inference_steps, end_scale=end_scale)
            elif method_type == 'mmsa_es' and i >= end_step:
                c.use_tca = False
            model_inputs = torch.cat([lat, lat], dim=1).reshape(4 * E, C, h, w)
            c.log_mask = False
            noise_pred = self._unet(model_inputs, t, text_embeddings)
            out = self.cfg_ctrl_step(noise_pred, t, lat.reshape(2 * E, C, h, w), local_cfg_reg if local_text_edit else None,
                                     var_mask, guidance_scale, eta=eta)
            edit = out.reshape(E, 2, C, h, w)[:, 0]
            latents_list.append(edit if E > 1 else edit[0])
            last = out
        image = self.latent2image(last, return_type="pt")
        if return_intermediates:
            return image, latents_list
        return image, None

    def Details_Preserving_regeneration_background(self, ori_img, inverted_latents, edit_prompt, ori_mask, num_steps=100,
                                                   start_step=30, end_step=10, guidance_scale=3.5, eta=1, verbose=False,
                                                   local_text_edit=True, local_perturbation=True, end_scale=0.5,
                                                   return_intermediates=False, share_attn=True, method_type='tca',
                                                   latent_blended=True, blend_range=(0, 40)):
        init_code_orig = deepcopy(inverted_latents[-1])
        full_h, full_w = ori_img.shape[:2]
        mask_tensor, local_var_reg = self.prepare_mask_bggen(ori_mask, full_h, full_w, init_code_orig)
        c = self.controller
        c.fg_retain_mask = mask_tensor.to(self.device)
        c.local_edit_region = mask_tensor.to(self.device)
        c.reset()
        gen_images, intermediates = self.forward_sampling_background_gen(
            prompt=[edit_prompt, ""], end_step=end_step, batch_size=2, refer_latents=inverted_latents[::-1],
            latents=init_code_orig, guidance_scale=guidance_scale, num_inference_steps=num_steps,
            num_actual_inference_steps=num_steps - start_step, eta=eta, local_cfg_reg=local_var_reg,
            local_var_reg=local_var_reg, share_attn=share_attn, method_type=method_type, verbose=verbose,
            local_text_edit=local_text_edit, local_perturbation=local_perturbation,
            return_intermediates=return_intermediates, end_scale=end_scale, latent_blended=latent_blended,
            blend_range=blend_range)
        c.reset()
        edit = (gen_images[0].permute(1, 2, 0).detach().cpu().numpy() * 255).astype(np.uint8)
        return edit, intermediates

    def FreeFine_background_generation(self, ori_img, ori_mask, guidance_text, guidance_scale, eta, end_step=10,
                                       num_step=50, start_step=25, share_attn=True, method_type='tca',
                                       local_text_edit=True, local_perturbation=True, verbose=True, seed=42,
                                       return_intermediates=False, end_scale=0.5, latent_blended=False,
                                       blend_range=(0, 40)):
        seed_everything(seed)
        ori_mask = self.mask_reduce_dim(ori_mask)
        _, inverted = self.DDIM_inversion_func(img=ori_img, mask=ori_mask, prompt="", num_step=num_step,
                                               start_step=start_step, ref_img=None, verbose=verbose)
        edit, intermediates = self.Details_Preserving_regeneration_background(
            ori_img, inverted, guidance_text, ori_mask, num_steps=num_step, start_step=start_step, end_step=end_step,
            guidance_scale=guidance_scale, eta=eta, share_attn=share_attn, method_type=method_type, verbose=verbose,
            end_scale=end_scale, local_text_edit=local_text_edit, local_perturbation=local_perturbation,
            return_intermediates=return_intermediates, latent_blended=latent_blended, blend_range=blend_range)
        self.last_intermediates = intermediates
        return edit

    def prepare_composition_masks(self, ori_mask_lists, tgt_mask_lists, sup_res_w, sup_res_h, init_code,
                                  dil_completion=False, dil_factor=15, draw_mask=None, appearance_transfer=False):
        P = lambda m: self.prepare_tensor_mask(m, sup_res_w, sup_res_h)
        lat = (init_code.shape[2], init_code.shape[3])
        down = lambda t: F.interpolate(t[None, None], lat, mode='nearest').squeeze(0).squeeze(0)
        ori = [P(m) for m in ori_mask_lists]
        tgt = []
        lp, fg = torch.zeros_like(ori[0]), torch.zeros_like(ori[0])
        if appearance_transfer:
            for shifted in tgt_mask_lists:
                d = P(self.dilate_mask(shifted, dil_factor))
                tgt.append(d)
                lp += d
            lp[lp > 0] = 1
            tgt.append(1 - lp)
            lp = down(lp)
            return torch.stack(tgt), torch.stack(ori), lp, deepcopy(lp)
        if draw_mask is None:
            for shifted in tgt_mask_lists:
                d = P(self.dilate_mask(shifted, dil_factor))
                sh = P(shifted)
                tgt.append(d if dil_completion else sh)
                fg += sh
                lp += d
            fg[fg > 0] = 1
            lp[lp > 0] = 1
            tgt.append(1 - fg if dil_completion else 1 - lp)
            lp = down(lp * (1 - fg))
            return torch.stack(tgt), torch.stack(ori), lp, (deepcopy(lp) if dil_completion else torch.zeros_like(lp))
        for i, shifted in enumerate(tgt_mask_lists):
            sh = P(shifted)
            d = P(draw_mask[i]) + sh
            d[d > 0] = 1
            tgt.append(d)
            fg += sh
            lp += d
        fg[fg > 0] = 1
        lp[lp > 0] = 1
        tgt.append(1 - lp)
        lp = down(lp * (1 - fg))
        return torch.stack(tgt), torch.stack(ori), lp, lp

    @torch.no_grad()
    def DDIM_inversion_func_compose(self, img, compose_imgs, prompt, num_step, start_step=0, verbose=False):
        source = torch.cat([self.preprocess_image(im, self.device) for im in [img] + list(compose_imgs)])
        _, latents_list = self.invert(source, prompt, guidance_scale=1.0, num_inference_steps=num_step,
                                      num_actual_inference_steps=num_step - start_step, return_intermediates=True,
                                      verbose=verbose)
        self.controller.reset()
        return latents_list

    @torch.no_grad()
    def forward_sampling_compose(self, prompt, prompt_embeds=None, refer_latents=None, batch_size=1, end_step=None,
                                 height=512, width=512, num_inference_steps=50, num_actual_inference_steps=None,
                                 guidance_scale=7.5, latents=None, unconditioning=None, neg_prompt=None,
                                 return_intermediates=False, eta=0.0, end_scale=0.5, local_var_reg=None,
                                 local_edit_text=True, cfg_masks_tensor=None, share_attn=True, method_type=None,
                                 verbose=False, local_perturbation=True, **kwds):
        self.method_type = method_type
        assert guidance_scale > 1.0, 'USING THIS MODULE CFG Must > 1.0'
        c = self.controller
        if share_attn:
            if method_type == 'tca':
                c.use_tca, c.layer_idx, c.method = True, list(range(10, 16)), 'tca'
            elif method_type in ('mmsa', 'mmsa_es'):
                c.use_tca, c.layer_idx, c.method = True, list(range(10, 16)), 'mmsa'
            elif method_type == 'ssa':
                c.use_style_align, c.method = True, 'ssa'
            elif method_type == 'sdsa':
                c.use_style_align, c.method = True, 'sdsa'
        c.use_cfg = True
        c.local_edit = local_edit_text
        prompt = list(prompt) + [""]
        c.prompt_length = len(prompt)
        cond = self.get_text_embeddings(prompt)
        n_lat = latents.shape[0]
        uncond = self.get_text_embeddings([neg_prompt if neg_prompt else ""] * n_lat)
        text_embeddings = torch.cat([uncond, cond], dim=0)
        self.scheduler.set_timesteps(num_inference_steps)
        if num_actual_inference_steps is None:
            num_actual_inference_steps = num_inference_steps
        start_step = num_inference_steps - num_actual_inference_steps
        C, h, w = latents.shape[1:]
        edit = latents.float()[:1]
        latents_list = [latents]
        var_mask = local_var_reg if local_perturbation else torch.ones_like(local_var_reg)
        for i, t in enumerate(self.scheduler.timesteps):
            if i < start_step:
                continue
            refs = refer_latents[i - start_step + 1][1:].float()
            if method_type == 'tca':
                c.context_guidance = self.linear_param(i, start_step, end_step, num_inference_steps, end_scale=end_scale)
            elif method_type == 'mmsa_es' and i >= end_step:
                c.use_tca = False
            model_inputs = torch.cat([edit, refs, edit])
            c.log_mask = False
            noise_pred = self._unet(model_inputs, t, text_embeddings)
            noise = None
            if eta > 0:
                noise = randn_tensor(edit.shape, device=edit.device, dtype=torch.float32).contiguous()
            edit = ops.ddim_cfg_step_compose(noise_pred.contiguous(), model_inputs.shape[0], edit.contiguous(), noise,
                                             self._var_mask(cfg_masks_tensor, 1, h, w) if local_edit_text else None,
                                             self._var_mask(var_mask, 1, h, w), float(guidance_scale),
                                             **self._ctrl_coefs(t, eta))
            latents_list.append(edit[0])
        image = self.latent2image(edit, return_type="pt")[0]
        if return_intermediates:
            return image, latents_list
        return image, None

    @torch.no_grad()
    def Details_Preserving_regeneration_compose(self, source_image, inverted_latents, edit_prompt_list, ori_mask_lists,
                                                tgt_mask_lists, draw_mask, num_steps=100, start_step=30, end_step=10,
                                                eta=1, guidance_scale=7.5, dil_completion=False,
                                                appearance_transfer=False, share_attn=True, method_type='tca',
                                                verbose=False, local_text_edit=True, local_perturbation=True,
                                                return_intermediates=False, use_share_attention=False, dil_factor=15,
                                                end_scale=0.5):
        from ._lib import FF_MAX_PASS
        n_src = len(ori_mask_lists)
        if n_src + 1 > FF_MAX_PASS:
            raise ValueError(f"cross-image composition with {n_src} source images needs {n_src + 1} attention passes per "
                             f"head; this build supports FF_MAX_PASS = {FF_MAX_PASS} (at most {FF_MAX_PASS - 1} sources)")
        init_code_orig = deepcopy(inverted_latents[-1])
        full_h, full_w = source_image.shape[:2]
        tgt_masks, ori_masks, local_pert, comp_cfg = self.prepare_composition_masks(
            ori_mask_lists, tgt_mask_lists, full_h, full_w, init_code_orig, dil_completion=dil_completion,
            dil_factor=dil_factor, draw_mask=draw_mask, appearance_transfer=appearance_transfer)
        c = self.controller
        c.src_masks, c.tgt_masks = ori_masks.to(self.device), tgt_masks.to(self.device)
        c.reset()
        image, intermediates = self.forward_sampling_compose(
            prompt=edit_prompt_list, refer_latents=inverted_latents[::-1], end_step=end_step,
            batch_size=init_code_orig.shape[0], latents=init_code_orig, guidance_scale=guidance_scale,
            num_inference_steps=num_steps, num_actual_inference_steps=num_steps - start_step, eta=eta,
            local_var_reg=local_pert, local_edit_text=local_text_edit, cfg_masks_tensor=comp_cfg, share_attn=share_attn,
            method_type=method_type, verbose=verbose, local_perturbation=local_perturbation,
            return_intermediates=return_intermediates, use_share_attention=use_share_attention, end_scale=end_scale)
        c.reset()
        return (image.permute(1, 2, 0).detach().cpu().numpy() * 255).astype(np.uint8), intermediates

    def FreeFine_cross_image_composition(self, img_lists, ori_mask_lists, tgt_mask_lists, coarse_input,
                                         guidance_text_list, guidance_scale, eta, end_step=10, num_step=50,
                                         start_step=25, share_attn=True, method_type='tca', local_text_edit=True,
                                         local_perturbation=True, verbose=True, seed=42, draw_mask=None,
                                         return_intermediates=False, use_auto_draw=False, end_scale=0.5,
                                         dil_completion=False, dil_factor=15, appearance_transfer=False):
        methods = ['tca', 'ssa', 'sdsa', 'mmsa', 'mmsa_es']
        assert method_type in methods, f"check method type f{method_type}, which is not in {methods}"
        seed_everything(seed)
        ori_mask_lists = [self.mask_reduce_dim(m) for m in ori_mask_lists]
        tgt_mask_lists = [self.mask_reduce_dim(m) for m in tgt_mask_lists]
        inverted = self.DDIM_inversion_func_compose(img=coarse_input, compose_imgs=img_lists, prompt="", num_step=num_step,
                                                    start_step=start_step, verbose=verbose)
        image, intermediates = self.Details_Preserving_regeneration_compose(
            coarse_input, inverted, guidance_text_list, ori_mask_lists, tgt_mask_lists, draw_mask, num_steps=num_step,
            start_step=start_step, end_step=end_step, dil_factor=dil_factor, guidance_scale=guidance_scale, eta=eta,
            share_attn=share_attn, method_type=method_type, verbose=verbose, dil_completion=dil_completion,
            local_text_edit=local_text_edit, local_perturbation=local_perturbation,
            return_intermediates=return_intermediates, end_scale=end_scale, appearance_transfer=appearance_transfer)
        self.last_intermediates = intermediates
        return image

    def prepare_various_mask_batch(self, shifted, ori, draw, cons, lat_hw, use_auto_draw, reduce_inp_artifacts):
        if shifted.is_cuda:
            need_cons = use_auto_draw or reduce_inp_artifacts
            return ops.mask_prep(shifted.contiguous(), ori.contiguous(), None if use_auto_draw else draw.contiguous(),
                                 cons.contiguous() if need_cons else None, lat_hw, use_auto_draw, reduce_inp_artifacts)
        b = lambda t: (t > 0).to(torch.uint8)

        def dil(t, k):
            a = k // 2
            x = F.pad(b(t)[:, None].float(), (a, k - 1 - a, a, k - 1 - a), value=0.0)
            return F.max_pool2d(x, kernel_size=k, stride=1)[:, 0].to(torch.uint8)

        sh, orim = b(shifted), b(ori)
        if not use_auto_draw:
            flex = b(draw) * (1 - sh)
            fg = flex + sh
            fg[fg > 0] = 1
            comp = flex
            if not reduce_inp_artifacts:
                lvar = flex
            else:
                lvar = (1 - b(cons)) * (1 - sh) * dil(ori, 30) + flex
                lvar[lvar > 0] = 1
        else:
            fg = sh
            c2 = b(cons) - orim
            if not reduce_inp_artifacts:
                comp = (1 - c2) * (1 - sh) * dil(shifted, 15)
            else:
                comp = dil(ori, 30) + dil(shifted, 15)
                comp[comp > 0] = 1
                comp = comp * ((1 - c2) * (1 - sh))
            lvar = comp
        ds = lambda t: F.interpolate(t[:, None], lat_hw, mode='nearest')[:, 0].contiguous()
        return fg, sh, orim, ds(comp), ds(lvar)

    @torch.no_grad()
    def FreeFine_generation_batch(self, ori_imgs, ori_masks, edit_params, guidance_texts, guidance_scale=7.5, eta=1.0,
                                  end_step=50, num_step=50, start_step=35, method_type='tca', seed=42, draw_masks=None,
                                  use_auto_draw=True, reduce_inp_artifacts=True, end_scale=0.0, inp_bgs=None,
                                  thetas=None, return_latents=False, coarse_inputs=None, target_masks=None):
        from . import coarse_edit
        assert method_type in ['tca', 'mmsa', 'mmsa_es'], method_type
        seed_everything(seed)
        host_in = not (torch.is_tensor(ori_imgs) and ori_imgs.is_cuda)
        to_dev = lambda a: (a if torch.is_tensor(a) else torch.from_numpy(np.ascontiguousarray(a))).to(self.device, non_blocking=True)
        imgs_u8, masks = to_dev(ori_imgs), to_dev(ori_masks)
        E, H, W = masks.shape
        if (coarse_inputs is None) != (target_masks is None):
            raise ValueError("coarse_inputs and target_masks go together")
        if coarse_inputs is None and thetas is None:
            mh = ori_masks.cpu().numpy() if torch.is_tensor(ori_masks) else np.asarray(ori_masks)
            thetas = torch.tensor(np.stack([coarse_edit.cv2_theta(coarse_edit.edit_matrix(mh[e], edit_params[e]), W, H)
                                            for e in range(E)]), dtype=torch.float32)
        imgs = imgs_u8.permute(0, 3, 1, 2).float().contiguous()
        bgs = imgs if inp_bgs is None else to_dev(inp_bgs).permute(0, 3, 1, 2).float().contiguous()
        if coarse_inputs is not None:
            coarse = to_dev(coarse_inputs).permute(0, 3, 1, 2).float().contiguous()
            tgt = to_dev(target_masks).contiguous()
        else:
            with ops.nvtx_range("ff.coarse_edit (warp + blend)"):
                coarse, tgt = coarse_edit.re_edit_2d_device(imgs, masks.contiguous(), to_dev(thetas), bgs)
            coarse = coarse.round().clamp(0, 255)
        draw = torch.zeros_like(masks) if draw_masks is None else to_dev(draw_masks)
        lat_hw = (H // 8, W // 8)
        fg, sh, orim, comp, lvar = self.prepare_various_mask_batch(tgt, masks, draw, tgt, lat_hw, use_auto_draw,
                                                                   reduce_inp_artifacts)
        src = torch.stack([coarse, imgs], dim=1).reshape(2 * E, 3, H, W) / 127.5 - 1
        _, inverted = self.invert(src, [""] * (2 * E), guidance_scale=1.0, num_inference_steps=num_step,
                                  num_actual_inference_steps=num_step - start_step, return_intermediates=True)
        c = self.controller
        c.reset()
        c.fg_retain_mask, c.fg_retain_mask_st2, c.fg_ref_mask, c.local_edit_region = fg, sh, orim, fg
        prompts = [p for t in guidance_texts for p in (t, "")]
        gens = [torch.Generator(device=self.device).manual_seed(int(seed)) for _ in range(E)] if eta > 0 else None
        image, inter = self.forward_sampling(prompt=prompts, refer_latents=inverted[::-1], end_step=end_step, generator=gens,
                                             latents=inverted[-1].clone(), guidance_scale=guidance_scale,
                                             num_inference_steps=num_step, num_actual_inference_steps=num_step - start_step,
                                             eta=eta, completion_mask_cfg=comp, local_var_reg=lvar, method_type=method_type,
                                             end_scale=end_scale, return_intermediates=True, verbose=True)
        c.reset()
        out = (image.view(E, 2, 3, H, W)[:, 0].permute(0, 2, 3, 1) * 255).to(torch.uint8)
        if host_in:
            out = out.cpu().numpy()
        if return_latents:
            return out, inter[-1]
        return out


__all__ = ["FreeFinePipeline", "Attention_Modulator", "register_attention_control",
           "register_attention_control_4bggen", "register_attention_control_compose", "randn_tensor"]
```

freefine_b200/plans.py:

```python
from __future__ import annotations

import numpy as np

from ._lib import (FF_MAX_PASS, FF_PASS_KEY2_INVERT, FF_PASS_KEY2_PREFIX, FF_PASS_KEY_INVERT, FF_PASS_KEY_PREFIX,
                   FF_PASS_ROW_WEIGHT, FF_PASS_ROW_XOR, PLAN_BYTES)

PASS_DTYPE = np.dtype([("kv_stream", "<i4"), ("key_mask", "<i4"), ("row_mask", "<i4"), ("flags", "<u4"),
                       ("weight", "<f4"), ("kv_stream2", "<i4"), ("key_mask2", "<i4"), ("reserved", "<i4")])
PLAN_DTYPE = np.dtype([("n_pass", "<i4"), ("reserved", "<i4", (3,)), ("passes", PASS_DTYPE, (FF_MAX_PASS,))])
assert PLAN_DTYPE.itemsize == PLAN_BYTES


def q0_masked(heads: int, stream_in_edit: int, head: int) -> bool:
    return ((heads * stream_in_edit + head) % 4) in (0, 2)


def _empty(n_streams: int, heads: int) -> np.ndarray:
    p = np.zeros((n_streams, heads), PLAN_DTYPE)
    p["passes"]["kv_stream"] = -1
    p["passes"]["kv_stream2"] = -1
    p["passes"]["key_mask"] = -1
    p["passes"]["key_mask2"] = -1
    p["passes"]["row_mask"] = -1
    return p


def _add(plan, s, h, kv, weight, key_mask=-1, row_mask=-1, flags=0, kv2=-1, key_mask2=-1):
    e = plan[s, h]
    i = int(e["n_pass"])
    if i >= FF_MAX_PASS:
        raise ValueError(f"more than {FF_MAX_PASS} passes for stream {s} head {h}")
    ps = e["passes"][i]
    ps["kv_stream"], ps["key_mask"], ps["row_mask"], ps["flags"] = kv, key_mask, row_mask, flags
    ps["weight"], ps["kv_stream2"], ps["key_mask2"] = weight, kv2, key_mask2
    plan[s, h]["n_pass"] = i + 1


def plain_plan(n_streams: int, heads: int, kv_of=None) -> np.ndarray:
    p = _empty(n_streams, heads)
    for s in range(n_streams):
        for h in range(heads):
            _add(p, s, h, s if kv_of is None else kv_of(s), 1.0)
    return p


def tca_plan(n_edits: int, heads: int, method: str, cg, src_id, tgt_id, kind: str = "edit",
             prefix: bool = False) -> np.ndarray:
    pf = FF_PASS_KEY_PREFIX if prefix else 0
    if method not in ("tca", "mmsa"):
        raise ValueError(f"method must be 'tca' or 'mmsa', got {method!r}")
    if kind not in ("edit", "bg"):
        raise ValueError(kind)
    p = _empty(4 * n_edits, heads)
    w_ref = 1.0 if method == "mmsa" else float(cg)
    w_self = 0.0 if method == "mmsa" else 1.0 - float(cg)
    for e in range(n_edits):
        for sl in range(4):
            s = 4 * e + sl
            r = 4 * e + (1 if sl < 2 else 3)
            for h in range(heads):
                masked = q0_masked(heads, sl, h)
                if not masked and r == s:
                    _add(p, s, h, s, 1.0 if method == "mmsa" else w_ref + w_self)
                    continue
                if masked and kind == "edit":
                    _add(p, s, h, r, w_ref, key_mask=src_id(e), row_mask=tgt_id(e),
                         flags=FF_PASS_KEY_INVERT | FF_PASS_ROW_XOR | pf)
                elif masked:
                    _add(p, s, h, r, w_ref, key_mask=src_id(e), flags=FF_PASS_KEY_INVERT | pf)
                else:
                    _add(p, s, h, r, w_ref)
                if method == "tca":
                    _add(p, s, h, s, w_self)
    return p


def compose_plan(n_src: int, heads: int, method: str, cg, src_ids, tgt_ids, prefix: bool = False) -> np.ndarray:
    if method not in ("tca", "mmsa"):
        raise ValueError(method)
    B = n_src + 2
    p = _empty(B, heads)
    for s in range(B):
        for h in range(heads):
            if s in (0, B - 1):
                w_new = 1.0 if method == "mmsa" else float(cg)
                for i in range(n_src):
                    _add(p, s, h, 1 + i, w_new, key_mask=src_ids[i], row_mask=tgt_ids[i],
                         flags=FF_PASS_ROW_WEIGHT | (FF_PASS_KEY_PREFIX if prefix else 0))
                if method == "tca":
                    _add(p, s, h, s, 1.0 - float(cg))
            else:
                _add(p, s, h, s, 1.0)
    return p


def style_align_plan(n_edits: int, heads: int, src_id=None, prefix: bool = False, bg: bool = False) -> np.ndarray:
    p = _empty(4 * n_edits, heads)
    for e in range(n_edits):
        for sl in range(4):
            s = 4 * e + sl
            r = 4 * e + (1 if sl < 2 else 3)
            for h in range(heads):
                masked = src_id is not None and q0_masked(heads, sl, h)
                if bg and masked:
                    _add(p, s, h, r, 1.0, key_mask=src_id(e), flags=FF_PASS_KEY_INVERT | (FF_PASS_KEY_PREFIX if prefix else 0))
                    continue
                km2 = src_id(e) if masked else -1
                _add(p, s, h, s, 1.0, kv2=r, key_mask2=km2, flags=FF_PASS_KEY2_PREFIX if (prefix and km2 >= 0) else 0)
    return p


def kv_sort_index(key_bits, stream_masks) -> "torch.Tensor":
    import torch
    n, S = key_bits.shape
    order = torch.sort(key_bits.to(torch.uint8), dim=1, descending=True, stable=True).indices
    ident = torch.arange(S, device=key_bits.device)
    rows = [order[m] if m >= 0 else ident for m in stream_masks]
    base = (torch.arange(len(stream_masks), device=key_bits.device) * S)[:, None]
    return (torch.stack(rows) + base).reshape(-1)


def algorithmic_flops(plan: np.ndarray, s_q: int, s_kv: int, d: int, popcount=None) -> float:
    total = 0.0
    for e in plan.reshape(-1):
        for ps in e["passes"][: int(e["n_pass"])]:
            flags = int(ps["flags"])
            n_r = int(popcount[int(ps["row_mask"])]) if ps["row_mask"] >= 0 else 0
            if ps["key_mask"] >= 0:
                n_k = int(popcount[int(ps["key_mask"])])
                c0 = s_kv - n_k if flags & FF_PASS_KEY_INVERT else n_k
            else:
                c0 = s_kv
            if flags & FF_PASS_ROW_WEIGHT:
                pairs = n_r * c0
            elif flags & FF_PASS_ROW_XOR and ps["key_mask"] >= 0:
                pairs = (s_q - n_r) * c0 + n_r * (s_kv - c0)
            else:
                pairs = s_q * c0
            if ps["kv_stream2"] >= 0:
                if ps["key_mask2"] >= 0:
                    n2 = int(popcount[int(ps["key_mask2"])])
                    pairs += s_q * (s_kv - n2 if flags & FF_PASS_KEY2_INVERT else n2)
                else:
                    pairs += s_q * s_kv
            total += 4.0 * d * pairs
    return total


def describe(plan: np.ndarray) -> str:
    out = []
    for s in range(plan.shape[0]):
        for h in range(plan.shape[1]):
            e = plan[s, h]
            ps = ", ".join(
                f"kv{int(q['kv_stream'])}" + (f"+kv{int(q['kv_stream2'])}" if q["kv_stream2"] >= 0 else "") +
                f"[k{int(q['key_mask'])} r{int(q['row_mask'])} f{int(q['flags'])}]*{float(q['weight']):.3f}"
                for q in e["passes"][: int(e["n_pass"])])
            out.append(f"s{s}h{h}: {ps}")
    return "\n".join(out)


__all__ = ["PASS_DTYPE", "PLAN_DTYPE", "q0_masked", "plain_plan", "tca_plan", "compose_plan", "style_align_plan",
           "kv_sort_index", "algorithmic_flops", "describe", "FF_PASS_KEY_INVERT", "FF_PASS_ROW_XOR", "FF_PASS_ROW_WEIGHT",
           "FF_PASS_KEY2_INVERT", "FF_PASS_KEY_PREFIX", "FF_PASS_KEY2_PREFIX"]
```

include/freefine_b200.h:

```cpp
#ifndef FREEFINE_B200_H_
#define FREEFINE_B200_H_

#include <stdint.h>

#ifdef __cplusplus
extern "C" {
#endif

#define FF_VERSION 100

enum {
  FF_OK = 0,
  FF_E_INVALID = -1,
  FF_E_UNSUPPORTED = -2,
  FF_E_CUDA = -3,
  FF_E_ARCH = -4
};

enum { FF_DT_F32 = 0, FF_DT_BF16 = 1, FF_DT_F16 = 2 };

int ff_version(void);
const char* ff_last_error(void);

#define FF_MAX_PASS 4

enum {
  FF_PASS_KEY_INVERT = 1u,
  FF_PASS_ROW_XOR = 2u,
  FF_PASS_ROW_WEIGHT = 4u,
  FF_PASS_KEY2_INVERT = 8u,
  FF_PASS_KEY_PREFIX = 16u,
  FF_PASS_KEY2_PREFIX = 32u
};

typedef struct FFAttnPass {
  int32_t kv_stream;
  int32_t key_mask;
  int32_t row_mask;
  uint32_t flags;
  float weight;
  int32_t kv_stream2;
  int32_t key_mask2;
  int32_t reserved;
} FFAttnPass;

typedef struct FFAttnHeadPlan {
  int32_t n_pass;
  int32_t reserved[3];
  FFAttnPass pass[FF_MAX_PASS];
} FFAttnHeadPlan;

typedef struct FFAttnArgs {
  const void* q;
  const void* k;
  const void* v;
  void* out;
  const FFAttnHeadPlan* plan;
  const uint32_t* bitmasks;
  const int32_t* mask_popcount;
  int32_t n_streams, n_kv_streams, heads, head_dim;
  int32_t s_q, s_kv;
  int32_t n_masks, mask_words;
  int32_t out_dtype;
  float scale;
  int32_t v_dtype;
  int32_t v_head_stride;
} FFAttnArgs;

int ff_attn_masked_kv(const FFAttnArgs* h_args, void* stream);

int ff_attn_plain_smallkv(const void* q, const void* k, const void* v, void* out, int32_t n_streams, int32_t heads,
                          int32_t head_dim, int32_t s_q, int32_t s_kv, float scale, int32_t out_dtype, void* stream);

int ff_attn_v_head_stride(int32_t head_dim);

int ff_kv_gather_cast(const void* k, const void* v, const int64_t* row_index, void* k_out, void* v_out,
                      int32_t v_out_dtype, int64_t rows, int32_t heads, int32_t head_dim, void* stream);

int ff_mask_downsample_pack(const uint8_t* masks, int32_t n, int32_t H, int32_t W, int32_t h, int32_t w,
                            uint32_t* bits, int32_t words, int32_t* popcount, void* stream);

int ff_mask_prep(const uint8_t* shifted, const uint8_t* ori, const uint8_t* draw, const uint8_t* cons, int32_t E,
                 int32_t H, int32_t W, int32_t h, int32_t w, int32_t use_auto_draw, int32_t reduce_inp_artifacts,
                 uint8_t* fg, uint8_t* shifted_out, uint8_t* ori_out, uint8_t* comp_lat, uint8_t* lvar_lat, void* stream);

int ff_dilate_mask(const uint8_t* mask, uint8_t* out, int32_t N, int32_t H, int32_t W, int32_t k, void* stream);

int ff_upsample2x_nhwc(const void* x, void* y, int32_t N, int32_t H, int32_t W, int32_t C, void* stream);
int ff_concat_nhwc(const void* a, const void* b, void* out, int64_t M, int32_t Ca, int32_t Cb, void* stream);

int ff_linear_bias_residual(const void* x, const void* w, const void* bias, const void* res, void* out, int64_t M, int32_t N,
                            int32_t K, void* workspace, int64_t ws_bytes, void* stream);

int ff_warp_affine_blend(const void* src, const float* theta, const uint8_t* mask_src, const void* bg, void* out,
                         uint8_t* mask_out, int32_t N, int32_t C, int32_t H, int32_t W, int32_t dH, int32_t dW,
                         int32_t mode, int32_t dtype, void* stream);

int ff_ddim_cfg_step(const float* eps4, const float* x, const float* noise, const uint8_t* cfg_mask,
                     const uint8_t* var_mask, float guidance_scale, float sqrt_1m_at, float sqrt_at, float sqrt_ap,
                     float c_ddim, float c_ddpm, float sigma, float* x_prev, float* pred_x0, int32_t n_edits,
                     int32_t C, int32_t h, int32_t w, void* stream);

int ff_ddim_step(const float* eps2, const float* x, const float* noise, const uint8_t* var_mask, float sqrt_1m_at,
                 float sqrt_at, float sqrt_ap, float c_ddim, float c_ddpm, float sigma, float* x_prev,
                 float* pred_x0, int32_t n_edits, int32_t C, int32_t h, int32_t w, void* stream);

int ff_ddim_cfg_step_compose(const float* eps, int32_t streams_per_edit, const float* x, const float* noise,
                             const uint8_t* cfg_mask, const uint8_t* var_mask, float guidance_scale, float sqrt_1m_at,
                             float sqrt_at, float sqrt_ap, float c_ddim, float c_ddpm, float sigma, float* x_prev,
                             float* pred_x0, int32_t n_edits, int32_t C, int32_t h, int32_t w, void* stream);

int ff_ddim_inv_step(const float* eps, const float* x, float sqrt_1m_at, float sqrt_at, float sqrt_an, float c_next,
                     float* x_next, float* pred_x0, int64_t n, void* stream);

int ff_cross_region_blend(void* hs, const uint32_t* bitmasks, int32_t mask_words, const int32_t* region_mask,
                          int32_t n_edits, int32_t S, int32_t C, int32_t dtype, void* stream);


int64_t ff_group_norm_ws_bytes(int32_t N, int32_t G);
int ff_group_norm_nhwc(const void* x, const float* add_nc, int64_t add_ld, const void* gamma, const void* beta, void* y,
                       void* workspace, int32_t N, int32_t HW, int32_t C, int32_t G, float eps, int32_t silu, void* stream);

int ff_bias_residual_nhwc(const void* h, const void* bias, const void* res, void* out, int64_t M, int32_t C,
                          void* stream);

int ff_geglu(const void* h, void* out, int64_t M, int32_t F, void* stream);

int ff_layer_norm(const void* x, const void* gamma, const void* beta, void* y, int64_t M, int32_t C, float eps,
                  void* stream);

int ff_debug_set_trace(void* device_visible_ptr);
int ff_debug_set_timeline(void* device_ptr);

#ifdef __cplusplus
}
#endif
#endif
```

Before: 2.778.

## Drop duplicate stream in sampling batch: three streams per edit instead of four

Reduces the UNet sampling batch from four streams per edit [u_e,u_r,c_e,c_r] to three, sharing one reference stream between the unconditional and conditional branches. The attention plans, KV index, cross-region blend kernel and DDIM CFG step kernel are extended to handle the 3-stream layout through a separate reference-offset argument. The aim is to cut a quarter of UNet work per denoising step. The risk is that the conditional reference branch now uses the shared reference stream's output, which could change results if that stream would otherwise have differed, for example through its text embedding.

```diff
diff --git a/freefine_b200/_lib.py b/freefine_b200/_lib.py
--- a/freefine_b200/_lib.py
+++ b/freefine_b200/_lib.py
@@ -54,6 +54,9 @@
     "ff_ddim_cfg_step": (C.c_int, [C.c_void_p, C.c_void_p, C.c_void_p, C.c_void_p, C.c_void_p, C.c_float, C.c_float,
                                    C.c_float, C.c_float, C.c_float, C.c_float, C.c_float, C.c_void_p, C.c_void_p,
                                    C.c_int32, C.c_int32, C.c_int32, C.c_int32, C.c_void_p]),
+    "ff_ddim_cfg_step3": (C.c_int, [C.c_void_p, C.c_void_p, C.c_void_p, C.c_void_p, C.c_void_p, C.c_float, C.c_float,
+                                    C.c_float, C.c_float, C.c_float, C.c_float, C.c_float, C.c_void_p, C.c_void_p,
+                                    C.c_int32, C.c_int32, C.c_int32, C.c_int32, C.c_void_p]),
     "ff_debug_set_trace": (C.c_int, [C.c_void_p]),
     "ff_ddim_step": (C.c_int, [C.c_void_p, C.c_void_p, C.c_void_p, C.c_void_p, C.c_float, C.c_float, C.c_float,
                                C.c_float, C.c_float, C.c_float, C.c_void_p, C.c_void_p, C.c_int32, C.c_int32,
@@ -65,6 +68,8 @@
                                    C.c_void_p, C.c_int64, C.c_void_p]),
     "ff_cross_region_blend": (C.c_int, [C.c_void_p, C.c_void_p, C.c_int32, C.c_void_p, C.c_int32, C.c_int32,
                                         C.c_int32, C.c_int32, C.c_void_p]),
+    "ff_cross_region_blend_streams": (C.c_int, [C.c_void_p, C.c_void_p, C.c_int32, C.c_void_p, C.c_int32, C.c_int32,
+                                                C.c_int32, C.c_int32, C.c_int32, C.c_void_p]),
     "ff_group_norm_ws_bytes": (C.c_int64, [C.c_int32, C.c_int32]),
     "ff_group_norm_nhwc": (C.c_int, [C.c_void_p, C.c_void_p, C.c_int64, C.c_void_p, C.c_void_p, C.c_void_p, C.c_void_p,
                                      C.c_int32, C.c_int32, C.c_int32, C.c_int32, C.c_float, C.c_int32, C.c_void_p]),
diff --git a/freefine_b200/attention.py b/freefine_b200/attention.py
--- a/freefine_b200/attention.py
+++ b/freefine_b200/attention.py
@@ -78,6 +78,7 @@
         self.src_masks = None
         self.tgt_masks = None
         self.prompt_length = 1
+        self.n_edits = None
         self.heads = None
         self.scale = None
         self.upcast_attention = False
@@ -106,6 +107,7 @@
         self.context_guidance = None
         self.tca_scope = ['up']
         self.style_align_scope = ['down', 'mid', 'up']
+        self.n_edits = None
         self._tables.clear()
         self._plans.clear()
 
@@ -158,8 +160,14 @@
             ops.PLAN_REGISTRY[p.data_ptr()] = host
         return p
 
+    def _layout(self, B: int, allowed=(3, 4)):
+        E = self.n_edits if self.n_edits is not None else B // 4
+        if E <= 0 or B % E or B // E not in allowed:
+            raise ValueError(f"a batch of {B} streams for n_edits={self.n_edits} is not {allowed} streams per edit")
+        return E, B // E
+
     def _kv_index(self, kind: str, seq: int, bits, stream_masks):
-        ck = (kind, "kvidx", seq)
+        ck = (kind, "kvidx", seq, tuple(stream_masks))
         hit = self._tables.get(ck)
         if hit is not None and hit[0] is bits:
             return hit[1]
@@ -202,11 +210,9 @@
             out = self.plain_attention(query, key, value)
             self._advance()
             return out
-        if B % 4:
-            raise ValueError(f"TCA expects 4 streams [u_e,u_r,c_e,c_r] per edit, got batch {B}")
+        E, spe = self._layout(B)
         if self.method not in ('tca', 'mmsa'):
             raise ValueError(f"controller.method must be 'tca' or 'mmsa' here, got {self.method!r}")
-        E = B // 4
         self._device = query.device
         if kind == "edit":
             bits, pop = self._table("edit", S, [self.fg_ref_mask, self.fg_retain_mask])
@@ -218,11 +224,12 @@
             raise ValueError(f"{E} edits in the stream batch but masks for {bits.shape[0]} rows")
         cg = None if self.method == 'mmsa' else float(self.context_guidance)
         pf = self.sort_keys
-        plan = self._plan((kind, E, self.heads, self.method, cg, pf),
-                          lambda: plans.tca_plan(E, self.heads, self.method, cg, src_id, tgt_id, kind=kind, prefix=pf))
+        plan = self._plan((kind, E, spe, self.heads, self.method, cg, pf),
+                          lambda: plans.tca_plan(E, self.heads, self.method, cg, src_id, tgt_id, kind=kind, prefix=pf,
+                                                 streams_per_edit=spe))
         kv_index = None
         if pf:
-            kv_index = self._kv_index(kind, S, bits, [src_id(s // 4) if s % 2 else -1 for s in range(B)])
+            kv_index = self._kv_index(kind, S, bits, [src_id(s // spe) if (s % spe) % 2 else -1 for s in range(B)])
         out = self._attend(query, key, value, plan, bits, pop, kv_index)
         self._advance()
         return out
@@ -281,15 +288,14 @@
 
     def modulate_local_cross_attn(self, query, key, value, is_cross, place_in_unet):
         B, S, _ = query.shape
-        if B % 4:
-            raise ValueError("local cross-attention modulation expects 4 streams per edit")
+        E, spe = self._layout(B, allowed=(2, 3, 4))
         hs = self.plain_attention(query, key, value)
         bits, _ = self._table("region", S, [self.local_edit_region])
-        ids = self._plans.get(("region_ids", B // 4))
+        ids = self._plans.get(("region_ids", E))
         if ids is None:
-            ids = torch.arange(B // 4, dtype=torch.int32, device=query.device)
-            self._plans[("region_ids", B // 4)] = ids
-        ops.cross_region_blend(hs, bits, ids)
+            ids = torch.arange(E, dtype=torch.int32, device=query.device)
+            self._plans[("region_ids", E)] = ids
+        ops.cross_region_blend(hs, bits, ids, streams_per_edit=spe)
         self._advance()
         return hs
 
diff --git a/freefine_b200/csrc/cross_blend.cu b/freefine_b200/csrc/cross_blend.cu
--- a/freefine_b200/csrc/cross_blend.cu
+++ b/freefine_b200/csrc/cross_blend.cu
@@ -4,9 +4,10 @@
 
 __global__ void __launch_bounds__(256)
 cross_region_blend_kernel(uint4* __restrict__ hs, const uint32_t* __restrict__ bitmasks, int mask_words,
-                          const int* __restrict__ region_mask, int n_edits, int S, int row_vec) {
+                          const int* __restrict__ region_mask, int n_edits, int spe, int S, int row_vec) {
   const long long per_stream = (long long)S * row_vec;
   const long long total = (long long)n_edits * per_stream;
+  const int ce = spe == 2 ? 1 : 2;
   for (long long i = (long long)blockIdx.x * blockDim.x + threadIdx.x; i < total;
        i += (long long)gridDim.x * blockDim.x) {
     const int e = (int)(i / per_stream);
@@ -14,11 +15,33 @@
     const int tok = (int)(r / row_vec);
     const uint32_t word = __ldg(bitmasks + (size_t)__ldg(region_mask + e) * mask_words + (tok >> 5));
     const bool in_region = (word >> (tok & 31)) & 1u;
-    uint4* base = hs + (long long)e * 4 * per_stream + r;
-    const uint4 ur = base[per_stream];
-    if (!in_region) base[2 * per_stream] = base[0];
-    base[3 * per_stream] = ur;
+    uint4* base = hs + (long long)e * spe * per_stream + r;
+    if (spe == 4) {
+      const uint4 ur = base[per_stream];
+      if (!in_region) base[2 * per_stream] = base[0];
+      base[3 * per_stream] = ur;
+    } else if (!in_region) {
+      base[ce * per_stream] = base[0];
+    }
   }
+}
+
+int launch_blend(const char* what, void* hs, const uint32_t* bitmasks, int32_t mask_words, const int32_t* region_mask,
+                 int32_t n_edits, int32_t spe, int32_t S, int32_t C, int32_t dtype, void* stream) {
+  FF_REQUIRE(hs && bitmasks && region_mask, "%s: null pointer", what);
+  FF_REQUIRE(n_edits > 0 && S > 0 && C > 0, "%s: bad shape", what);
+  FF_REQUIRE(spe == 2 || spe == 3 || spe == 4, "%s: streams_per_edit must be 2, 3 or 4, got %d", what, spe);
+  FF_REQUIRE(dtype == FF_DT_F32 || dtype == FF_DT_BF16, "%s: dtype must be f32 or bf16", what);
+  const int es = dtype == FF_DT_F32 ? 4 : 2;
+  FF_REQUIRE((C * es) % 16 == 0 && ff::aligned16(hs), "%s: rows must be 16-byte multiples", what);
+  FF_REQUIRE(mask_words >= (S + 31) / 32, "%s: mask_words too small", what);
+  const int row_vec = C * es / 16;
+  const long long total = (long long)n_edits * S * row_vec;
+  long long grid = (total + 255) / 256;
+  if (grid > 148 * 8) grid = 148 * 8;
+  cross_region_blend_kernel<<<(int)grid, 256, 0, static_cast<cudaStream_t>(stream)>>>(
+      static_cast<uint4*>(hs), bitmasks, mask_words, region_mask, n_edits, spe, S, row_vec);
+  return ff::check_launch(what);
 }
 
 }
@@ -26,17 +49,12 @@
 extern "C" int ff_cross_region_blend(void* hs, const uint32_t* bitmasks, int32_t mask_words,
                                      const int32_t* region_mask, int32_t n_edits, int32_t S, int32_t C, int32_t dtype,
                                      void* stream) {
-  FF_REQUIRE(hs && bitmasks && region_mask, "ff_cross_region_blend: null pointer");
-  FF_REQUIRE(n_edits > 0 && S > 0 && C > 0, "ff_cross_region_blend: bad shape");
-  FF_REQUIRE(dtype == FF_DT_F32 || dtype == FF_DT_BF16, "ff_cross_region_blend: dtype must be f32 or bf16");
-  const int es = dtype == FF_DT_F32 ? 4 : 2;
-  FF_REQUIRE((C * es) % 16 == 0 && ff::aligned16(hs), "ff_cross_region_blend: rows must be 16-byte multiples");
-  FF_REQUIRE(mask_words >= (S + 31) / 32, "ff_cross_region_blend: mask_words too small");
-  const int row_vec = C * es / 16;
-  const long long total = (long long)n_edits * S * row_vec;
-  long long grid = (total + 255) / 256;
-  if (grid > 148 * 8) grid = 148 * 8;
-  cross_region_blend_kernel<<<(int)grid, 256, 0, static_cast<cudaStream_t>(stream)>>>(
-      static_cast<uint4*>(hs), bitmasks, mask_words, region_mask, n_edits, S, row_vec);
-  return ff::check_launch("ff_cross_region_blend");
+  return launch_blend("ff_cross_region_blend", hs, bitmasks, mask_words, region_mask, n_edits, 4, S, C, dtype, stream);
 }
+
+extern "C" int ff_cross_region_blend_streams(void* hs, const uint32_t* bitmasks, int32_t mask_words,
+                                             const int32_t* region_mask, int32_t n_edits, int32_t streams_per_edit,
+                                             int32_t S, int32_t C, int32_t dtype, void* stream) {
+  return launch_blend("ff_cross_region_blend_streams", hs, bitmasks, mask_words, region_mask, n_edits, streams_per_edit,
+                      S, C, dtype, stream);
+}
diff --git a/freefine_b200/csrc/ddim_step.cu b/freefine_b200/csrc/ddim_step.cu
--- a/freefine_b200/csrc/ddim_step.cu
+++ b/freefine_b200/csrc/ddim_step.cu
@@ -30,7 +30,7 @@
 ddim_cfg_step_kernel(const float* __restrict__ eps4, const float* __restrict__ x, const float* __restrict__ noise,
                      const uint8_t* __restrict__ cfg_mask, const uint8_t* __restrict__ var_mask, StepCoef k,
                      float* __restrict__ x_prev, float* __restrict__ pred_x0, int n_edits, int C, int hw, int spe,
-                     int so, int cs) {
+                     int so, int cs, int cs_ref) {
   const int hwv = hw / V;
   const long long total = (long long)n_edits * so * C * hwv;
   for (long long i = (long long)blockIdx.x * blockDim.x + threadIdx.x; i < total;
@@ -42,7 +42,7 @@
     const int s = so == 2 ? (int)(r & 1) : 0;
     const int e = so == 2 ? (int)(r >> 1) : (int)r;
     const long long off_u = (((long long)(e * spe + s) * C + c) * hw) + (long long)p * V;
-    const long long off_c = (((long long)(e * spe + s + cs) * C + c) * hw) + (long long)p * V;
+    const long long off_c = (((long long)(e * spe + s + (s == 0 ? cs : cs_ref)) * C + c) * hw) + (long long)p * V;
     const long long off_x = (((long long)(e * so + s) * C + c) * hw) + (long long)p * V;
     const long long off_m = (long long)e * hw + (long long)p * V;
     float eu[V], ec[V], xv[V], nz[V], xp[V], x0[V];
@@ -120,7 +120,8 @@
 
 }
 
-static int launch_step(const char* what, const float* eps, int spe, int so, int cs, const float* x, const float* noise,
+static int launch_step(const char* what, const float* eps, int spe, int so, int cs, int cs_ref, const float* x,
+                       const float* noise,
                        const uint8_t* cfg_mask, const uint8_t* var_mask, const StepCoef& k, float* x_prev,
                        float* pred_x0, int32_t n_edits, int32_t C, int32_t h, int32_t w, void* stream) {
   if (!(eps && x && var_mask && x_prev)) return ff::fail(FF_E_INVALID, "%s: null pointer", what);
@@ -135,11 +136,11 @@
   if (vec) {
     const long long items = (long long)n_edits * so * C * (hw / 4);
     ddim_cfg_step_kernel<4><<<grid_for(items, 256), 256, 0, st>>>(eps, x, noise, cfg_mask, var_mask, k, x_prev,
-                                                                   pred_x0, n_edits, C, hw, spe, so, cs);
+                                                                   pred_x0, n_edits, C, hw, spe, so, cs, cs_ref);
   } else {
     const long long items = (long long)n_edits * so * C * hw;
     ddim_cfg_step_kernel<1><<<grid_for(items, 256), 256, 0, st>>>(eps, x, noise, cfg_mask, var_mask, k, x_prev,
-                                                                   pred_x0, n_edits, C, hw, spe, so, cs);
+                                                                   pred_x0, n_edits, C, hw, spe, so, cs, cs_ref);
   }
   return ff::check_launch(what);
 }
@@ -149,8 +150,17 @@
                                 float sqrt_ap, float c_ddim, float c_ddpm, float sigma, float* x_prev,
                                 float* pred_x0, int32_t n_edits, int32_t C, int32_t h, int32_t w, void* stream) {
   StepCoef k{guidance_scale, sqrt_1m_at, sqrt_at, sqrt_ap, c_ddim, c_ddpm, sigma};
-  return launch_step("ff_ddim_cfg_step", eps4, 4, 2, 2, x, noise, cfg_mask, var_mask, k, x_prev, pred_x0, n_edits, C, h,
+  return launch_step("ff_ddim_cfg_step", eps4, 4, 2, 2, 2, x, noise, cfg_mask, var_mask, k, x_prev, pred_x0, n_edits, C, h,
                      w, stream);
+}
+
+extern "C" int ff_ddim_cfg_step3(const float* eps3, const float* x, const float* noise, const uint8_t* cfg_mask,
+                                 const uint8_t* var_mask, float guidance_scale, float sqrt_1m_at, float sqrt_at,
+                                 float sqrt_ap, float c_ddim, float c_ddpm, float sigma, float* x_prev,
+                                 float* pred_x0, int32_t n_edits, int32_t C, int32_t h, int32_t w, void* stream) {
+  StepCoef k{guidance_scale, sqrt_1m_at, sqrt_at, sqrt_ap, c_ddim, c_ddpm, sigma};
+  return launch_step("ff_ddim_cfg_step3", eps3, 3, 2, 2, 0, x, noise, cfg_mask, var_mask, k, x_prev, pred_x0, n_edits, C,
+                     h, w, stream);
 }
 
 extern "C" int ff_ddim_step(const float* eps2, const float* x, const float* noise, const uint8_t* var_mask,
@@ -158,7 +168,7 @@
                             float* x_prev, float* pred_x0, int32_t n_edits, int32_t C, int32_t h, int32_t w,
                             void* stream) {
   StepCoef k{0.f, sqrt_1m_at, sqrt_at, sqrt_ap, c_ddim, c_ddpm, sigma};
-  return launch_step("ff_ddim_step", eps2, 2, 2, 0, x, noise, nullptr, var_mask, k, x_prev, pred_x0, n_edits, C, h, w,
+  return launch_step("ff_ddim_step", eps2, 2, 2, 0, 0, x, noise, nullptr, var_mask, k, x_prev, pred_x0, n_edits, C, h, w,
                      stream);
 }
 
@@ -169,7 +179,7 @@
                                         int32_t w, void* stream) {
   FF_REQUIRE(streams_per_edit >= 2, "ff_ddim_cfg_step_compose: streams_per_edit=%d < 2", streams_per_edit);
   StepCoef k{guidance_scale, sqrt_1m_at, sqrt_at, sqrt_ap, c_ddim, c_ddpm, sigma};
-  return launch_step("ff_ddim_cfg_step_compose", eps, streams_per_edit, 1, streams_per_edit - 1, x, noise, cfg_mask,
+  return launch_step("ff_ddim_cfg_step_compose", eps, streams_per_edit, 1, streams_per_edit - 1, 0, x, noise, cfg_mask,
                      var_mask, k, x_prev, pred_x0, n_edits, C, h, w, stream);
 }
 
diff --git a/freefine_b200/ops.py b/freefine_b200/ops.py
--- a/freefine_b200/ops.py
+++ b/freefine_b200/ops.py
@@ -70,8 +70,9 @@
     _chk(x, torch.float32, "x")
     Cc, h, w = x.shape[-3:]
     n_edits = x.numel() // (2 * Cc * h * w)
-    if eps4.numel() != 2 * x.numel():
-        raise ValueError(f"eps4 {tuple(eps4.shape)} must hold 4 streams per edit for x {tuple(x.shape)}")
+    if 2 * eps4.numel() not in (4 * x.numel(), 3 * x.numel()):
+        raise ValueError(f"eps4 {tuple(eps4.shape)} must hold 4 or 3 streams per edit for x {tuple(x.shape)}")
+    entry = "ff_ddim_cfg_step" if eps4.numel() == 2 * x.numel() else "ff_ddim_cfg_step3"
     _chk(var_mask, torch.uint8, "var_mask")
     if var_mask.numel() != n_edits * h * w:
         raise ValueError("var_mask must be [n_edits,h,w]")
@@ -86,11 +87,11 @@
     x_prev = torch.empty_like(x) if out is None else _chk(out, torch.float32, "out")
     x0 = torch.empty_like(x) if want_pred_x0 else None
     lib = _lib.load()
-    rc = lib.ff_ddim_cfg_step(_ptr(eps4), _ptr(x), _ptr(noise), _ptr(cfg_mask), _ptr(var_mask), guidance_scale,
-                              sqrt_1m_at, sqrt_at, sqrt_ap, c_ddim, c_ddpm, sigma, _ptr(x_prev), _ptr(x0), n_edits,
-                              Cc, h, w, _stream())
-    _lib.check(rc, "ff_ddim_cfg_step")
-    _count("ff_ddim_cfg_step")
+    rc = getattr(lib, entry)(_ptr(eps4), _ptr(x), _ptr(noise), _ptr(cfg_mask), _ptr(var_mask), guidance_scale,
+                             sqrt_1m_at, sqrt_at, sqrt_ap, c_ddim, c_ddpm, sigma, _ptr(x_prev), _ptr(x0), n_edits,
+                             Cc, h, w, _stream())
+    _lib.check(rc, entry)
+    _count(entry)
     return (x_prev, x0) if want_pred_x0 else x_prev
 
 
@@ -349,19 +350,29 @@
     return out
 
 
-def cross_region_blend(hs, bitmasks, region_ids):
+def cross_region_blend(hs, bitmasks, region_ids, streams_per_edit=4):
     if hs.dtype not in _DT:
         raise TypeError("hs must be float32 or bfloat16")
     _chk(hs, hs.dtype, "hs", 3)
     B, S, Cc = hs.shape
-    if B % 4:
-        raise ValueError("hs must hold 4 streams per edit")
+    if streams_per_edit not in (2, 3, 4) or B % streams_per_edit:
+        raise ValueError(f"hs with {B} streams does not hold {streams_per_edit} streams per edit")
     _chk(bitmasks, torch.int32, "bitmasks", 2)
     _chk(region_ids, torch.int32, "region_ids", 1)
-    rc = _lib.load().ff_cross_region_blend(_ptr(hs), _ptr(bitmasks), bitmasks.shape[1], _ptr(region_ids), B // 4, S, Cc,
-                                           _DT[hs.dtype], _stream())
-    _lib.check(rc, "ff_cross_region_blend")
-    _count("ff_cross_region_blend")
+    E = B // streams_per_edit
+    if region_ids.numel() < E:
+        raise ValueError(f"region_ids must hold one mask row per edit ({E}), got {region_ids.numel()}")
+    lib = _lib.load()
+    if streams_per_edit == 4:
+        rc = lib.ff_cross_region_blend(_ptr(hs), _ptr(bitmasks), bitmasks.shape[1], _ptr(region_ids), E, S, Cc,
+                                       _DT[hs.dtype], _stream())
+        entry = "ff_cross_region_blend"
+    else:
+        rc = lib.ff_cross_region_blend_streams(_ptr(hs), _ptr(bitmasks), bitmasks.shape[1], _ptr(region_ids), E,
+                                               streams_per_edit, S, Cc, _DT[hs.dtype], _stream())
+        entry = "ff_cross_region_blend_streams"
+    _lib.check(rc, entry)
+    _count(entry)
     return hs
 
 
diff --git a/freefine_b200/pipeline.py b/freefine_b200/pipeline.py
--- a/freefine_b200/pipeline.py
+++ b/freefine_b200/pipeline.py
@@ -222,11 +222,14 @@
         if n2 % 2:
             raise ValueError("forward_sampling expects [edit_prompt, \"\"] pairs")
         E = n2 // 2
+        c.n_edits = E
         if latents is None:
             latents = torch.randn((n2, self.unet.in_channels, height // 8, width // 8), device=self.device)
         uncond = self.get_text_embeddings([neg_prompt if neg_prompt else ""] * n2)
+        spe = 3 if (method_type in ('tca', 'mmsa', 'mmsa_es') and local_edit_text) else 4
+        slots = [0, 1, 2] if spe == 3 else [0, 1, 2, 3]
         text_embeddings = torch.cat([uncond.reshape(E, 2, *uncond.shape[1:]), cond.reshape(E, 2, *cond.shape[1:])],
-                                    dim=1).reshape(4 * E, *cond.shape[1:])
+                                    dim=1)[:, slots].reshape(spe * E, *cond.shape[1:])
         self.scheduler.set_timesteps(num_inference_steps)
         latents = latents.float().clone()
         latents_list = [latents]
@@ -249,12 +252,12 @@
             elif method_type == 'mmsa_es' and i >= end_step:
                 c.use_tca = False
             lat = latents.view(E, 2, C, h, w)
-            model_inputs = torch.cat([lat, lat], dim=1).reshape(4 * E, C, h, w)
+            model_inputs = torch.cat([lat, lat], dim=1)[:, slots].reshape(spe * E, C, h, w)
             te = text_embeddings
             if unconditioning is not None and isinstance(unconditioning, list):
-                te = text_embeddings.clone().reshape(E, 4, *cond.shape[1:])
+                te = text_embeddings.clone().reshape(E, spe, *cond.shape[1:])
                 te[:, :2] = unconditioning[i].to(te.dtype)
-                te = te.reshape(4 * E, *cond.shape[1:])
+                te = te.reshape(spe * E, *cond.shape[1:])
             c.log_mask = False
             with ops.nvtx_range(f"ff.sample step {i} t={int(t)}"):
                 noise_pred = self._unet(model_inputs, t, te)
@@ -464,6 +467,7 @@
                 c.use_style_align, c.method = True, 'sdsa'
         c.use_cfg = True
         c.local_edit = local_text_edit
+        c.n_edits = None
         if isinstance(prompt, str) and batch_size > 1:
             prompt = [prompt] * batch_size
         cond = self.get_text_embeddings(prompt)
diff --git a/freefine_b200/plans.py b/freefine_b200/plans.py
--- a/freefine_b200/plans.py
+++ b/freefine_b200/plans.py
@@ -45,19 +45,24 @@
 
 
 def tca_plan(n_edits: int, heads: int, method: str, cg, src_id, tgt_id, kind: str = "edit",
-             prefix: bool = False) -> np.ndarray:
+             prefix: bool = False, streams_per_edit: int = 4) -> np.ndarray:
     pf = FF_PASS_KEY_PREFIX if prefix else 0
     if method not in ("tca", "mmsa"):
         raise ValueError(f"method must be 'tca' or 'mmsa', got {method!r}")
     if kind not in ("edit", "bg"):
         raise ValueError(kind)
-    p = _empty(4 * n_edits, heads)
+    spe = streams_per_edit
+    if spe not in (3, 4):
+        raise ValueError(f"streams_per_edit must be 4 or 3, got {spe}")
+    if spe == 3 and heads % 2:
+        raise ValueError(f"the 3-stream layout needs an even head count (Q0 pattern of u_r and c_r), got {heads}")
+    p = _empty(spe * n_edits, heads)
     w_ref = 1.0 if method == "mmsa" else float(cg)
     w_self = 0.0 if method == "mmsa" else 1.0 - float(cg)
     for e in range(n_edits):
-        for sl in range(4):
-            s = 4 * e + sl
-            r = 4 * e + (1 if sl < 2 else 3)
+        for sl in range(spe):
+            s = spe * e + sl
+            r = spe * e + (1 if sl < 2 or spe == 3 else 3)
             for h in range(heads):
                 masked = q0_masked(heads, sl, h)
                 if not masked and r == s:
diff --git a/include/freefine_b200.h b/include/freefine_b200.h
--- a/include/freefine_b200.h
+++ b/include/freefine_b200.h
@@ -101,6 +101,11 @@
                      float c_ddim, float c_ddpm, float sigma, float* x_prev, float* pred_x0, int32_t n_edits,
                      int32_t C, int32_t h, int32_t w, void* stream);
 
+int ff_ddim_cfg_step3(const float* eps3, const float* x, const float* noise, const uint8_t* cfg_mask,
+                      const uint8_t* var_mask, float guidance_scale, float sqrt_1m_at, float sqrt_at, float sqrt_ap,
+                      float c_ddim, float c_ddpm, float sigma, float* x_prev, float* pred_x0, int32_t n_edits,
+                      int32_t C, int32_t h, int32_t w, void* stream);
+
 int ff_ddim_step(const float* eps2, const float* x, const float* noise, const uint8_t* var_mask, float sqrt_1m_at,
                  float sqrt_at, float sqrt_ap, float c_ddim, float c_ddpm, float sigma, float* x_prev,
                  float* pred_x0, int32_t n_edits, int32_t C, int32_t h, int32_t w, void* stream);
@@ -115,6 +120,9 @@
 
 int ff_cross_region_blend(void* hs, const uint32_t* bitmasks, int32_t mask_words, const int32_t* region_mask,
                           int32_t n_edits, int32_t S, int32_t C, int32_t dtype, void* stream);
+int ff_cross_region_blend_streams(void* hs, const uint32_t* bitmasks, int32_t mask_words, const int32_t* region_mask,
+                                  int32_t n_edits, int32_t streams_per_edit, int32_t S, int32_t C, int32_t dtype,
+                                  void* stream);
 
 
 int64_t ff_group_norm_ws_bytes(int32_t N, int32_t G);
diff --git a/profiles/sampling_call_profile.py b/profiles/sampling_call_profile.py
--- /dev/null
+++ b/profiles/sampling_call_profile.py
@@ -0,0 +1,97 @@
+#!/usr/bin/env python
+from __future__ import annotations
+
+import argparse
+import json
+import os
+import sys
+import time
+
+ROOT = os.path.dirname(os.path.dirname(os.path.abspath(__file__)))
+sys.path.insert(0, ROOT)
+
+
+def main():
+    ap = argparse.ArgumentParser()
+    ap.add_argument("--out", required=True)
+    ap.add_argument("--edits", type=int, default=8)
+    ap.add_argument("--res", type=int, default=512)
+    ap.add_argument("--start-step", type=int, default=0)
+    args = ap.parse_args()
+    import numpy as np
+    import torch
+    from torch.profiler import ProfilerActivity, profile
+    from freefine_b200 import _lib, coarse_edit, synth
+    from freefine_b200.pipeline import Attention_Modulator, FreeFinePipeline, register_attention_control
+    from freefine_b200.standin import build_standin
+
+    if not torch.cuda.is_available():
+        raise SystemExit("needs a CUDA device")
+    dev = torch.device("cuda:0")
+    _lib.load()
+    torch.backends.cudnn.benchmark = True
+    torch.backends.cuda.matmul.allow_tf32 = True
+    torch.backends.cudnn.allow_tf32 = True
+    E, R = args.edits, args.res
+    parts = build_standin("sd15", device=dev, dtype=torch.bfloat16)
+    c = Attention_Modulator(start_layer=10)
+    pipe = FreeFinePipeline.from_parts(parts, c, device=dev)
+    register_attention_control(pipe, c)
+    pipe.modify_unet_forward()
+    b = synth.make_batch(0, E, R)
+    thetas = torch.tensor(np.stack([coarse_edit.cv2_theta(coarse_edit.edit_matrix(b["masks"][i], b["edit_params"][i]), R, R)
+                                    for i in range(E)]), dtype=torch.float32).to(dev)
+    imgs, masks = torch.from_numpy(b["images"]).to(dev), torch.from_numpy(b["masks"]).to(dev)
+    kw = dict(guidance_scale=7.5, eta=1.0, end_step=50, num_step=50, start_step=args.start_step, method_type="tca",
+              use_auto_draw=True, reduce_inp_artifacts=True, end_scale=0.0)
+    run = lambda: pipe.FreeFine_generation_batch(imgs, masks, None, b["prompts"], thetas=thetas, **kw)
+
+    for _ in range(2):
+        run()
+    torch.cuda.synchronize()
+    torch.cuda.reset_peak_memory_stats()
+    t0 = time.perf_counter()
+    run()
+    torch.cuda.synchronize()
+    batch_s = time.perf_counter() - t0
+    peak = torch.cuda.max_memory_allocated()
+
+    orig = pipe._unet
+    cap = {"armed": True}
+
+    def unet(latents, t, te):
+        if cap["armed"] and latents.shape[0] > 2 * E:
+            cap["armed"] = False
+            torch.cuda.synchronize()
+            with profile(activities=[ProfilerActivity.CUDA]) as prof:
+                out = orig(latents, t, te)
+                torch.cuda.synchronize()
+            cap["prof"], cap["streams"] = prof, int(latents.shape[0])
+            return out
+        return orig(latents, t, te)
+
+    pipe._unet = unet
+    run()
+    torch.cuda.synchronize()
+    ks = [e for e in cap["prof"].events() if getattr(e, "device_type", None) is not None and str(e.device_type).endswith("CUDA")
+          and e.time_range is not None]
+    table = {}
+    for e in ks:
+        d = table.setdefault(e.name, [0, 0.0])
+        d[0] += 1
+        d[1] += float(e.time_range.end - e.time_range.start)
+    rows = sorted(({"kernel": k[:160], "launches": v[0], "total_us": round(v[1], 1)} for k, v in table.items()),
+                  key=lambda r: -r["total_us"])
+    res = {"edits": E, "res": R, "start_step": args.start_step, "sampling_call_streams": cap["streams"],
+           "kernel_launches": len(ks), "kernel_time_ms": sum(r["total_us"] for r in rows) / 1e3,
+           "device_span_ms": (max(e.time_range.end for e in ks) - min(e.time_range.start for e in ks)) / 1e3,
+           "batch_wall_s": batch_s, "max_memory_allocated_bytes": int(peak),
+           "gpu": torch.cuda.get_device_name(dev), "kernels": rows}
+    os.makedirs(args.out, exist_ok=True)
+    with open(os.path.join(args.out, "sampling_call_profile.json"), "w") as f:
+        json.dump(res, f, indent=1)
+    print(json.dumps({k: v for k, v in res.items() if k != "kernels"}))
+
+
+if __name__ == "__main__":
+    main()
```

After: 3.267 (median of 6 runs). 1.18x the previous value.
